# Corv/CUDA-GMM-MPI

Measured on NVIDIA H100. Metric: EM iterations/sec at N=10M D=24 K=64; E-step HBM GB/s vs roofline, higher is better.
Workload: dtype f32

## Files before the change

### cuda-gmm-mpi_b200/csrc/kernels_tc.cu

```cuda
#include <cuda.h>
#include <cudaTypedefs.h>
#include <cuda_fp16.h>
#if defined(__F16C__) && defined(__AVX__)
#include <immintrin.h>
#endif
#include <cuda_runtime.h>

#include <cmath>
#include <cstdio>
#include <cstdlib>
#include <cstring>
#include <string>
#include <vector>

#include "host_math.h"
#include "kernels_tc.cuh"
#include "tc_ptx.cuh"

namespace gmm {

using namespace ptx;

#define TC_CUDA_TRY(expr)                                                                     \
    do {                                                                                      \
        cudaError_t e_ = (expr);                                                              \
        if (e_ != cudaSuccess)                                                                \
            return fail(GMM_ERR_CUDA, std::string(#expr) + ": " + cudaGetErrorString(e_));    \
    } while (0)

constexpr int kTE = 32;
constexpr int kNCL = 32;
constexpr int kNST = 3;
constexpr int kNRAW = 4;
constexpr int kChunkSub = 4;
constexpr int kChunkSub2 = 16;
constexpr int kPhiBits = 11;
constexpr float kGammaScale = 1024.0f;
constexpr float kGammaMagic = 1.5f * 134217728.0f;

template <int D> struct MCfg {
    static_assert(D % 4 == 0, "tensor M-step: D must be a multiple of 4");
    static constexpr int F = 1 + D + D * (D + 1) / 2;
    static constexpr int S = D / 4;
    static constexpr int RPP = 1 + 2 * S + S * (D / 2);
    static constexpr int CPP = (RPP + 7) / 8;
    static constexpr int NCHUNK = 4 * CPP;
    static constexpr int MT = (NCHUNK * 8 + 127) / 128;
    static constexpr int PHI_PART = NCHUNK * 8 * kTE * 2;
    static constexpr int PHI_STAGE = 2 * PHI_PART;
    static constexpr int G_PART = kNCL * kTE * 2;
    static constexpr int G_STAGE = 3 * G_PART;
    static constexpr int RAWX = D * kTE * 4;
    static constexpr int RAWG = kNCL * kTE * 4;
    static constexpr int OFF_PHI = 0;
    static constexpr int OFF_G = OFF_PHI + kNST * PHI_STAGE;
    static constexpr int OFF_RAWX = OFF_G + kNST * G_STAGE;
    static constexpr int OFF_RAWG = OFF_RAWX + kNRAW * RAWX;
    static constexpr int NCT = MT * 128;
    static constexpr int OFF_RACC = OFF_RAWG + kNRAW * RAWG;
    static constexpr int OFF_BAR = OFF_RACC + 32 * NCT * 4;
    static constexpr int SMEM_BYTES = OFF_BAR + 512;
    static constexpr int THREADS = 384 + NCT;
    static constexpr int REG_LAUNCH = (65536 / THREADS) / 8 * 8 > 255 ? 255 : (65536 / THREADS) / 8 * 8;
    static constexpr int REG_P = MT == 1 ? 40 : 24;
    static constexpr int REG_B = MT == 3 ? 80 : 112;
    static constexpr int REG_C = MT == 3 ? 96 : (MT == 2 ? 112 : 240);
    static_assert(128 * REG_P + 256 * REG_B + NCT * REG_C <= THREADS * REG_LAUNCH, "register pools");
    static_assert(OFF_RAWG % 1024 == 0 && RAWG % 1024 == 0, "SWIZZLE_128B TMA destinations need 1024-byte alignment");
    static_assert((MT * 128 - NCHUNK * 8) * kTE * 2 <= kNST * G_STAGE, "the last part's over-read stays inside the operand stages");
    static_assert(MT <= 3, "feature tiles");
};

template <int R, int L>
__device__ __forceinline__ void set_regs() {
    if constexpr (R < L) asm volatile("setmaxnreg.dec.sync.aligned.u32 %0;" ::"n"(R));
    else if constexpr (R > L) asm volatile("setmaxnreg.inc.sync.aligned.u32 %0;" ::"n"(R));
}

struct MMagic { float lin, prod; };

__host__ __device__ constexpr int tri_row(int t) {
    int i = 0;
    while ((i + 1) * (i + 2) / 2 <= t) i++;
    return i;
}

__device__ __forceinline__ void tma_load_2d(void* smem_dst, const CUtensorMap* tmap, int c0, int c1, uint64_t* bar) {
    asm volatile(
        "cp.async.bulk.tensor.2d.shared::cluster.global.mbarrier::complete_tx::bytes [%0], [%1, {%2, %3}], [%4];"
        ::"r"(smem_u32(smem_dst)), "l"(reinterpret_cast<uint64_t>(tmap)), "r"(c0), "r"(c1), "r"(smem_u32(bar)) : "memory");
}

template <int D>
__device__ __forceinline__ void feature_split(const float (&z)[D], int r, const MMagic& mg, float& h, float& l) {
    using C = MCfg<D>;
    if (r == 0) { h = 1.0f; l = 0.0f; }
    else if (r <= C::S) {
        const float v = z[r - 1];
        h = __fsub_rn(__fadd_rn(v, mg.lin), mg.lin);
        l = __fsub_rn(v, h);
    } else if (r < C::RPP) {
        int a, b;
        if (r <= 2 * C::S) { a = r - 1 - C::S; b = a; }
        else { const int t = r - 1 - 2 * C::S; a = t / (D / 2); b = (a + 1 + t % (D / 2)) % D; }
        h = __fsub_rn(__fmaf_rn(z[a], z[b], mg.prod), mg.prod);
        l = __fmaf_rn(z[a], z[b], -h);
    } else { h = 0.0f; l = 0.0f; }
}

template <int D>
__device__ __forceinline__ void build_phi_chunks(const float (&z)[D], const MMagic& mg, uint8_t* hi_base, uint8_t* lo_base, int e, int part) {
    using C = MCfg<D>;
    const int eoff = part * (C::CPP * 512) + (e >> 3) * 128 + (e & 7) * 16;
#pragma unroll
    for (int c = 0; c < C::CPP; c++) {
        float hi[8], lo[8];
#pragma unroll
        for (int u = 0; u < 8; u++) feature_split<D>(z, c * 8 + u, mg, hi[u], lo[u]);
        uint4 h, l;
        h.x = pack_half2(hi[0], hi[1]); h.y = pack_half2(hi[2], hi[3]); h.z = pack_half2(hi[4], hi[5]); h.w = pack_half2(hi[6], hi[7]);
        l.x = pack_half2(lo[0], lo[1]); l.y = pack_half2(lo[2], lo[3]); l.z = pack_half2(lo[4], lo[5]); l.w = pack_half2(lo[6], lo[7]);
        *reinterpret_cast<uint4*>(hi_base + c * 512 + eoff) = h;
        *reinterpret_cast<uint4*>(lo_base + c * 512 + eoff) = l;
    }
}

struct RowInfo { int f, i, j; };
static RowInfo tc_row_info(int D, int row) {
    const int S = D / 4, RPP = 1 + 2 * S + S * (D / 2), CPP = (RPP + 7) / 8;
    const int p = row / (CPP * 8), r = row % (CPP * 8);
    RowInfo o{-1, -1, -1};
    if (p >= 4 || r >= RPP) return o;
    if (r == 0) { if (p == 0) o.f = 0; return o; }
    if (r <= S) { o.i = (r - 1 + p * S) % D; o.f = 1 + o.i; return o; }
    int a, b;
    if (r <= 2 * S) { a = r - 1 - S; b = a; }
    else { const int t = r - 1 - 2 * S; a = t / (D / 2); b = (a + 1 + t % (D / 2)) % D; }
    const int ta = (a + p * S) % D, tb = (b + p * S) % D;
    if (a != b && (b - a + D) % D == D / 2 && ta >= D / 2) return o;
    o.i = ta > tb ? ta : tb;
    o.j = ta > tb ? tb : ta;
    o.f = feat2(D, o.i, o.j);
    return o;
}

__device__ __forceinline__ bool chain_ends(int i, int mt, int nsub) { return ((i + mt) % kChunkSub) == kChunkSub - 1 || i == nsub - 1; }
__device__ __forceinline__ bool chain_starts(int i, int mt) { return i == 0 || ((i + mt) % kChunkSub) == 0; }
__device__ __forceinline__ bool chain2_ends(int i, int mt, int nsub) { return ((i + mt) % kChunkSub2) == kChunkSub2 - 1 || i == nsub - 1; }
__device__ __forceinline__ bool chain2_starts(int i, int mt) { return i == 0 || ((i + mt) % kChunkSub2) == 0; }

template <int D>
__global__ void __launch_bounds__(MCfg<D>::THREADS, 1)
mstep_tc_kernel(const __grid_constant__ CUtensorMap tm_x, const __grid_constant__ CUtensorMap tm_g, int n,
                float* __restrict__ scratch, int events_per_cta, const __grid_constant__ MMagic magic) {
    using C = MCfg<D>;
    extern __shared__ __align__(1024) uint8_t smem[];
    uint64_t* bars = reinterpret_cast<uint64_t*>(smem + C::OFF_BAR);
    uint64_t* raw_full = bars;
    uint64_t* raw_empty = bars + kNRAW;
    uint64_t* op_full = bars + 2 * kNRAW;
    uint64_t* op_empty = op_full + kNST;

    const int warp = threadIdx.x >> 5, lane = threadIdx.x & 31;
    const int e_begin = blockIdx.x * events_per_cta;
    const int e_end = min(n, e_begin + events_per_cta);
    const int nsub = (e_end - e_begin + kTE - 1) / kTE;
    const int k0 = blockIdx.y * kNCL;

    for (int i = threadIdx.x * 16; i < C::OFF_RAWX; i += C::THREADS * 16) *reinterpret_cast<uint4*>(smem + i) = make_uint4(0, 0, 0, 0);
    if (threadIdx.x == 0) {
        for (int s = 0; s < kNRAW; s++) { mbar_init(&raw_full[s], 1); mbar_init(&raw_empty[s], 4); }
        for (int s = 0; s < kNST; s++) { mbar_init(&op_full[s], 4); mbar_init(&op_empty[s], 4 * C::MT); }
        fence_mbar_init();
    }
    fence_proxy_async_smem();
    __syncthreads();

    if (warp < 4) {
        set_regs<C::REG_P, C::REG_LAUNCH>();
        if (warp == 0) {
            if (elect_one()) {
                for (int i = 0; i < nsub; i++) {
                    const int st = i % kNRAW, ph = (i / kNRAW) & 1;
                    mbar_wait_parked(&raw_empty[st], ph ^ 1, 500);
                    mbar_arrive_expect_tx(&raw_full[st], kTE * D * 4 + C::RAWG);
                    const int e0 = e_begin + i * kTE;
                    tma_load_2d(smem + C::OFF_RAWX + st * C::RAWX, &tm_x, e0, 0, &raw_full[st]);
                    tma_load_2d(smem + C::OFF_RAWG + st * C::RAWG, &tm_g, e0, k0, &raw_full[st]);
                }
            }
        }
    } else if (warp < 12) {
        set_regs<C::REG_B, C::REG_LAUNCH>();
        const int bwg = (warp - 4) >> 2;
        const int part = (warp - 4) & 3;
        const int bt = threadIdx.x - 128 - bwg * 128;
        for (int i = bwg; i < nsub; i += 2) {
            const int rs = i % kNRAW, rph = (i / kNRAW) & 1;
            const int os = i % kNST, oph = (i / kNST) & 1;
            mbar_wait_parked(&raw_full[rs], rph, 200);
            float z[D];
            {
                const float* xr = reinterpret_cast<const float*>(smem + C::OFF_RAWX + rs * C::RAWX) + lane;
                int dd = part * C::S;
#pragma unroll
                for (int d = 0; d < D; d++) { z[d] = xr[dd * kTE]; dd = dd + 1 == D ? 0 : dd + 1; }
            }
            uint4 gh, gl, gs;
            float gdep;
            {
                const int kg = bt >> 5, l = bt & 31;
                const int k = kg * 8 + (l & 7), ce = l >> 3;
                const uint8_t* grow = smem + C::OFF_RAWG + rs * C::RAWG + k * (kTE * 4);
                const float4 a = *reinterpret_cast<const float4*>(grow + (((2 * ce) ^ (k & 7)) << 4));
                const float4 b = *reinterpret_cast<const float4*>(grow + (((2 * ce + 1) ^ (k & 7)) << 4));
                const float g[8] = {a.x, a.y, a.z, a.w, b.x, b.y, b.z, b.w};
                gdep = a.x + b.x;
                float hi[8], lo[8];
#pragma unroll
                for (int u = 0; u < 8; u++) {
                    hi[u] = __fsub_rn(__fmaf_rn(g[u], kGammaScale, kGammaMagic), kGammaMagic);
                    lo[u] = __fmaf_rn(g[u], kGammaScale, -hi[u]);
                }
                gh = make_uint4(pack_half2(hi[0], hi[1]), pack_half2(hi[2], hi[3]), pack_half2(hi[4], hi[5]), pack_half2(hi[6], hi[7]));
                gl = make_uint4(pack_half2(lo[0], lo[1]), pack_half2(lo[2], lo[3]), pack_half2(lo[4], lo[5]), pack_half2(lo[6], lo[7]));
                gs = make_uint4(pack_half2(g[0] * kGammaScale, g[1] * kGammaScale), pack_half2(g[2] * kGammaScale, g[3] * kGammaScale),
                                pack_half2(g[4] * kGammaScale, g[5] * kGammaScale), pack_half2(g[6] * kGammaScale, g[7] * kGammaScale));
            }
            float dep = gdep;
#pragma unroll
            for (int d = 0; d < D; d++) dep += z[d];
            __syncwarp();
            if (lane == 0) mbar_arrive_after(&raw_empty[rs], dep);
            else asm volatile("" ::"f"(dep));
            mbar_wait_parked(&op_empty[os], oph ^ 1, 200);
            uint8_t* phi_hi = smem + C::OFF_PHI + os * C::PHI_STAGE;
            uint8_t* phi_lo = phi_hi + C::PHI_PART;
            build_phi_chunks<D>(z, magic, phi_hi, phi_lo, lane, part);
            {
                uint8_t* g_hi = smem + C::OFF_G + os * C::G_STAGE;
                const int kg = bt >> 5, l = bt & 31;
                *reinterpret_cast<uint4*>(g_hi + kg * 512 + l * 16) = gh;
                *reinterpret_cast<uint4*>(g_hi + C::G_PART + kg * 512 + l * 16) = gl;
                *reinterpret_cast<uint4*>(g_hi + 2 * C::G_PART + kg * 512 + l * 16) = gs;
            }
            fence_proxy_async_smem();
            __syncwarp();
            if (lane == 0) mbar_arrive(&op_full[os]);
        }
    } else {
        set_regs<C::REG_C, C::REG_LAUNCH>();
        const int mt = __shfl_sync(0xffffffffu, (warp - 12) >> 2, 0);
        const int ct = threadIdx.x - 384;
        const int wq = warp & 3, gid = lane >> 2, qd = lane & 3;
        float* racc = reinterpret_cast<float*>(smem + C::OFF_RACC) + ct;
#pragma unroll
        for (int j = 0; j < 32; j++) racc[j * C::NCT] = 0.0f;
        float ex[2][16], rm[2][16];
#pragma unroll
        for (int h = 0; h < 2; h++)
#pragma unroll
            for (int j = 0; j < 16; j++) { ex[h][j] = 0.0f; rm[h][j] = 0.0f; }
        int held = -1;
        for (int i = 0; i < nsub; i++) {
            const int os = i % kNST, oph = (i / kNST) & 1;
            mbar_wait_parked(&op_full[os], oph, 100);
            const uint32_t phi = smem_u32(smem + C::OFF_PHI + os * C::PHI_STAGE);
            const uint32_t gam = smem_u32(smem + C::OFF_G + os * C::G_STAGE);
            const bool new1 = chain_starts(i, mt), new2 = chain2_starts(i, mt);
            wgmma_fence();
#pragma unroll
            for (int h = 0; h < 2; h++) {
#pragma unroll
                for (int ks = 0; ks < kTE / 16; ks++) {
                    const uint64_t hdesc = make_smem_desc(gam + ks * 256,  128,  512);
                    const uint64_t ldesc = make_smem_desc(gam + C::G_PART + ks * 256, 128, 512);
                    const uint64_t sdesc = make_smem_desc(gam + 2 * C::G_PART + ks * 256, 128, 512);
                    const uint32_t arow = mt * 8192 + h * 4096 + ks * 256;
                    const uint64_t ah = make_smem_desc(phi + arow,  128,  512);
                    const uint64_t al = make_smem_desc(phi + C::PHI_PART + arow, 128, 512);
                    wgmma_m64n32k16_ss_tn(ex[h], ah, hdesc, ks > 0 || !new1);
                    wgmma_m64n32k16_ss_tn(rm[h], ah, ldesc, ks > 0 || !new2);
                    wgmma_m64n32k16_ss_tn(rm[h], al, sdesc);
                }
            }
            wgmma_commit();
            wgmma_wait<1>();
            __syncwarp();
            if (lane == 0 && held >= 0) mbar_arrive(&op_empty[held]);
            held = os;
            if (chain_ends(i, mt, nsub)) {
                wgmma_wait<0>();
                __syncwarp();
                if (lane == 0) mbar_arrive(&op_empty[os]);
                held = -1;
#pragma unroll
                for (int h = 0; h < 2; h++) {
#pragma unroll
                    for (int j = 0; j < 16; j++) racc[(h * 16 + j) * C::NCT] += ex[h][j];
                    asm volatile("" ::: "memory");
                }
                if (chain2_ends(i, mt, nsub)) {
#pragma unroll
                    for (int h = 0; h < 2; h++) {
#pragma unroll
                        for (int j = 0; j < 16; j++) racc[(h * 16 + j) * C::NCT] += rm[h][j];
                        asm volatile("" ::: "memory");
                    }
                }
            }
        }
        wgmma_wait<0>();
        float* my = scratch + (size_t)(blockIdx.y * gridDim.x + blockIdx.x) * C::MT * 128 * kNCL + (size_t)mt * 128 * kNCL;
#pragma unroll
        for (int h = 0; h < 2; h++)
#pragma unroll
            for (int j = 0; j < 16; j += 2) {
                const int row = h * 64 + wq * 16 + gid + 8 * ((j >> 1) & 1);
                const int col = (j >> 2) * 8 + 2 * qd;
                *reinterpret_cast<float2*>(my + (size_t)row * kNCL + col) =
                    make_float2(racc[(h * 16 + j) * C::NCT], racc[(h * 16 + j + 1) * C::NCT]);
            }
    }
}

__global__ void standardise_soa_kernel(const float* __restrict__ xs, float* __restrict__ zs, size_t pitch, int n, int D,
                                       const float* __restrict__ shift_f, const float* __restrict__ inv_scale_f) {
    const int d = blockIdx.y;
    const float s = shift_f[d], isc = inv_scale_f[d];
    const float* x = xs + (size_t)d * pitch;
    float* z = zs + (size_t)d * pitch;
    for (long long e = (long long)blockIdx.x * blockDim.x + threadIdx.x; e < n; e += (long long)gridDim.x * blockDim.x)
        z[e] = __fmul_rn(__fsub_rn(x[e], s), isc);
}

__global__ void __launch_bounds__(256)
mstep_tc_finalize_kernel(const float* __restrict__ scratch, int ncta_x, int MT, int K, int F, const int3* __restrict__ rowmap,
                         const double* __restrict__ scale, double* __restrict__ stats) {
    constexpr int NQ = 256 / kNCL;
    __shared__ double part[NQ][kNCL];
    const int3 rm = rowmap[blockIdx.x];
    if (rm.x < 0) return;
    const int mt = blockIdx.x / 128, row = blockIdx.x % 128;
    const int col = threadIdx.x & (kNCL - 1), q = threadIdx.x / kNCL;
    double fac = 1.0 / (double)kGammaScale;
    if (rm.y >= 0) fac *= scale[rm.y];
    if (rm.z >= 0) fac *= scale[rm.z];
    for (int ty = 0; ty * kNCL < K; ty++) {
        double s = 0;
        for (int cx = q; cx < ncta_x; cx += NQ)
            s += (double)scratch[(((size_t)(ty * ncta_x + cx) * MT + mt) * 128 + row) * kNCL + col];
        part[q][col] = s;
        __syncthreads();
        const int k = ty * kNCL + col;
        if (q == 0 && k < K) {
            double t = 0;
#pragma unroll
            for (int u = 0; u < NQ; u++) t += part[u][col];
            stats[(size_t)k * F + rm.x] += t * fac;
        }
        __syncthreads();
    }
}


template <int D> struct ECfg {
    static_assert(D % 8 == 0, "tensor E-step: D must be a multiple of 8");
    static constexpr int CP = D / 8;
    static constexpr int NLO = (CP + 1 + 1) / 2 * 2;
    static constexpr int NCHKB = CP + NLO;
    static constexpr int GB = 16;
    static constexpr int N = GB * 8;
    static constexpr int MAXSG = 64 / GB;
    static constexpr int B_BLOCK = NCHKB * N * 16;
    static constexpr int B_SG = CP * B_BLOCK;
    static constexpr int OFF_B = 0;
    static constexpr int OFF_CK = OFF_B + MAXSG * B_SG;
    static constexpr int OFF_SH = OFF_CK + 512;
    static constexpr int OFF_BAR = OFF_SH + 256;
    static constexpr int SMEM_BYTES = OFF_BAR + 64;
    static constexpr int NWG = 2;
    static constexpr int THREADS = 128 * NWG;
};

#ifndef GMM_ESTEP_CUT
#define GMM_ESTEP_CUT 0
#endif

template <int D>
__device__ __forceinline__ void tc_stage_operand(uint8_t* smem, const uint8_t* __restrict__ b_img, const float* __restrict__ ck,
                                                 const float* __restrict__ shift_f, const float* __restrict__ inv_scale_f, int NSG) {
    using C = ECfg<D>;
    uint64_t* b_full = reinterpret_cast<uint64_t*>(smem + C::OFF_BAR);
    float* ck_s = reinterpret_cast<float*>(smem + C::OFF_CK);
    float* sh_s = reinterpret_cast<float*>(smem + C::OFF_SH);
    if (threadIdx.x == 0) { mbar_init(b_full, 1); fence_mbar_init(); }
    if (threadIdx.x < 64) { ck_s[threadIdx.x] = ck[threadIdx.x] * 1.4426950408889634f; ck_s[64 + threadIdx.x] = ck[64 + threadIdx.x]; }
    if (threadIdx.x < D) { sh_s[threadIdx.x] = shift_f[threadIdx.x]; sh_s[32 + threadIdx.x] = inv_scale_f[threadIdx.x]; }
    __syncthreads();
    if (threadIdx.x == 0) {
        mbar_arrive_expect_tx(b_full, (uint32_t)NSG * C::B_SG);
        for (int g = 0; g < NSG * C::CP; g++) tma_load_1d(smem + C::OFF_B + g * C::B_BLOCK, b_img + (size_t)g * C::B_BLOCK, C::B_BLOCK, b_full);
    }
}

template <int D>
__device__ __forceinline__ void tc_split_rows(const float2 (&xa)[D / 8], const float2 (&xb)[D / 8], const float* sh_s, const float* isc_s,
                                              int qd, uint32_t (&zh)[D / 8][2], uint32_t (&zl)[D / 8][2]) {
#pragma unroll
    for (int j = 0; j < D / 8; j++) {
        const float s0 = sh_s[8 * j + 2 * qd], s1 = sh_s[8 * j + 2 * qd + 1];
        const float i0 = isc_s[8 * j + 2 * qd], i1 = isc_s[8 * j + 2 * qd + 1];
#pragma unroll
        for (int r = 0; r < 2; r++) {
            const float2 x = r ? xb[j] : xa[j];
            const float z0 = __fmul_rn(__fsub_rn(x.x, s0), i0), z1 = __fmul_rn(__fsub_rn(x.y, s1), i1);
            const __half2 h = __floats2half2_rn(z0, z1);
            const float2 f = __half22float2(h);
            zh[j][r] = *reinterpret_cast<const uint32_t*>(&h);
            zl[j][r] = pack_half2(z0 - f.x, z1 - f.y);
        }
    }
}

template <int D>
__device__ __forceinline__ void tc_issue_group(float (&acc)[32], const uint32_t (&zh)[D / 8][2], const uint32_t (&zl)[D / 8][2],
                                               uint32_t bsg, int c, int h, uint32_t ones) {
    using C = ECfg<D>;
    constexpr int CP = C::CP;
    constexpr uint32_t CH = C::N * 16;
    const uint32_t bb = bsg + (uint32_t)c * C::B_BLOCK + (uint32_t)h * (CH / 2);
    wgmma_fence();
#pragma unroll
    for (int j = c; j < CP; j++)
        wgmma_m64n64k16_rs(acc, zh[j][0], zh[j][1], zh[j][0], zh[j][1], make_smem_desc(bb + j * CH, CP * CH, 128), j > c);
#pragma unroll
    for (int p = c; p < CP + 1; p += 2) {
        const int x = p, y = p + 1;
        if (y <= CP) {
            const uint32_t yc = y < CP ? (uint32_t)y : 2u * CP;
            const uint32_t a2 = y < CP ? zl[y < CP ? y : 0][0] : ones, a3 = y < CP ? zl[y < CP ? y : 0][1] : ones;
            wgmma_m64n64k16_rs(acc, zl[x][0], zl[x][1], a2, a3, make_smem_desc(bb + x * CH, (yc - x) * CH, 128), true);
        } else {
            wgmma_m64n64k16_rs(acc, 0u, 0u, ones, ones, make_smem_desc(bb + c * CH, (2 * CP - c) * CH, 128), true);
        }
    }
}

template <int D, int NSG>
__device__ __forceinline__ void tc_tile_logits(const uint32_t (&zh)[D / 8][2], const uint32_t (&zl)[D / 8][2], uint32_t bsm,
                                               const float* ck_s, int qd, uint32_t ones, float (&lg)[ECfg<D>::MAXSG][8]) {
    using C = ECfg<D>;
    constexpr int CP = C::CP;
    float acc[2][32];
    tc_issue_group<D>(acc[0], zh, zl, bsm, 0, 0, ones);
    wgmma_commit();
#pragma unroll
    for (int sg = 0; sg < C::MAXSG; sg++) {
        if (sg >= NSG) {
#pragma unroll
            for (int u = 0; u < 8; u++) lg[sg][u] = -INFINITY;
            continue;
        }
        const uint32_t bsg = bsm + (uint32_t)sg * C::B_SG;
        float sq[32];
#pragma unroll
        for (int u = 0; u < 32; u++) sq[u] = 0.f;
#pragma unroll
        for (int c = 0; c < CP; c++) {
#pragma unroll
            for (int h = 0; h < 2; h++) {
                if (sg + 1 == NSG && c + 1 == CP && h == 1) {
                    wgmma_wait<0>();
                } else {
                    if (h == 0) tc_issue_group<D>(acc[1], zh, zl, bsg, c, 1, ones);
                    else if (c + 1 < CP) tc_issue_group<D>(acc[0], zh, zl, bsg, c + 1, 0, ones);
                    else tc_issue_group<D>(acc[0], zh, zl, bsg + C::B_SG, 0, 0, ones);
                    wgmma_commit();
                    wgmma_wait<1>();
                }
                wgmma_pin(acc[h]);
                const float(&a)[32] = acc[h];
#if GMM_ESTEP_CUT == 1
                sq[0] += a[0];
#else
#pragma unroll
                for (int i = 0; i < 8; i++) {
                    float& s0 = sq[16 * h + 2 * i];
                    float& s1 = sq[16 * h + 2 * i + 1];
                    s0 = fmaf(a[4 * i], a[4 * i], fmaf(a[4 * i + 1], a[4 * i + 1], s0));
                    s1 = fmaf(a[4 * i + 2], a[4 * i + 2], fmaf(a[4 * i + 3], a[4 * i + 3], s1));
                }
#endif
            }
        }
#if GMM_ESTEP_CUT == 1
        for (int u = 0; u < 8; u++) lg[sg][u] = sq[0];
        continue;
#endif
        float w[16];
        const bool b1 = qd & 1, b2 = (qd >> 1) & 1;
#pragma unroll
        for (int u = 0; u < 16; u++) {
            const float send = b1 ? sq[u] : sq[16 + u], keep = b1 ? sq[16 + u] : sq[u];
            w[u] = keep + __shfl_xor_sync(0xffffffffu, send, 1);
        }
#pragma unroll
        for (int u = 0; u < 8; u++) {
            const float send = b2 ? w[u] : w[8 + u], keep = b2 ? w[8 + u] : w[u];
            const float qv = keep + __shfl_xor_sync(0xffffffffu, send, 2);
            const int k = sg * C::GB + 8 * (qd & 1) + 4 * (qd >> 1) + (u >> 1);
            lg[sg][u] = fmaf(ck_s[64 + k], qv, ck_s[k]);
        }
    }
}

template <int D, int NSG>
__global__ void __launch_bounds__(ECfg<D>::THREADS, 1)
estep_tc_kernel(const float* __restrict__ x_aos, const uint8_t* __restrict__ b_img, const float* __restrict__ ck,
                const float* __restrict__ shift_f, const float* __restrict__ inv_scale_f, float* __restrict__ memb,
                size_t pitch, int n, int K, double* __restrict__ ll_out, int mode, const float* den_in, float* den_out) {
    using C = ECfg<D>;
    constexpr int CP = C::CP;
    extern __shared__ __align__(1024) uint8_t smem[];
    uint64_t* b_full = reinterpret_cast<uint64_t*>(smem + C::OFF_BAR);
    float* ck_s = reinterpret_cast<float*>(smem + C::OFF_CK);
    float* sh_s = reinterpret_cast<float*>(smem + C::OFF_SH);
    float* isc_s = sh_s + 32;

    const int wg = threadIdx.x >> 7, warp = (threadIdx.x >> 5) & 3, lane = threadIdx.x & 31;
    const int gid = lane >> 2, qd = lane & 3;
    const int ntiles = (n + 63) / 64;

    tc_stage_operand<D>(smem, b_img, ck, shift_f, inv_scale_f, NSG);

    const int r0 = warp * 16 + gid;
    float2 xa[CP], xb[CP];
    auto load_rows = [&](int t) {
        const long long e0 = (long long)t * 64 + r0, e1 = e0 + 8;
#pragma unroll
        for (int j = 0; j < CP; j++) {
            xa[j] = e0 < n ? __ldg(reinterpret_cast<const float2*>(x_aos + (size_t)e0 * D + 8 * j + 2 * qd)) : make_float2(0.f, 0.f);
            xb[j] = e1 < n ? __ldg(reinterpret_cast<const float2*>(x_aos + (size_t)e1 * D + 8 * j + 2 * qd)) : make_float2(0.f, 0.f);
        }
    };
    const int stride = (int)gridDim.x * C::NWG;
    int t = (int)blockIdx.x * C::NWG + wg;
    if (t < ntiles) load_rows(t);
    const uint32_t ones = qd == 0 ? 0x3C003C00u : 0u;
    const uint32_t bsm = smem_u32(smem + C::OFF_B);
    double ll_acc = 0.0;
    constexpr float kLn2 = 0.6931471805599453f;
    mbar_wait(b_full, 0);

    for (; t < ntiles; t += stride) {
        uint32_t zh[CP][2], zl[CP][2];
        tc_split_rows<D>(xa, xb, sh_s, isc_s, qd, zh, zl);
        const long long e0 = (long long)t * 64 + r0, e1 = e0 + 8;
        if (t + stride < ntiles) load_rows(t + stride);

        float lg[C::MAXSG][8];
        tc_tile_logits<D, NSG>(zh, zl, bsm, ck_s, qd, ones, lg);
#if GMM_ESTEP_CUT == 1
        for (int sg = 0; sg < C::MAXSG; sg++) ll_acc += (double)lg[sg][0];
        continue;
#endif
        float mx[2] = {-INFINITY, -INFINITY};
#pragma unroll
        for (int sg = 0; sg < C::MAXSG; sg++)
#pragma unroll
            for (int u = 0; u < 8; u++) mx[u & 1] = fmaxf(mx[u & 1], lg[sg][u]);
#pragma unroll
        for (int r = 0; r < 2; r++) {
            mx[r] = fmaxf(mx[r], __shfl_xor_sync(0xffffffffu, mx[r], 1));
            mx[r] = fmaxf(mx[r], __shfl_xor_sync(0xffffffffu, mx[r], 2));
        }
        float scale[2] = {1.f, 1.f};
        const long long er[2] = {e0, e1};
        if (mode == 3) {
            float d2[2];
#pragma unroll
            for (int r = 0; r < 2; r++) d2[r] = er[r] < n ? den_in[er[r]] * 1.4426950408889634f : 0.f;
#pragma unroll
            for (int sg = 0; sg < C::MAXSG; sg++)
#pragma unroll
                for (int u = 0; u < 8; u++) lg[sg][u] = ex2_approx(lg[sg][u] - d2[u & 1]);
        } else {
            float sm[2] = {0.f, 0.f};
#pragma unroll
            for (int sg = 0; sg < C::MAXSG; sg++)
#pragma unroll
                for (int u = 0; u < 8; u++) { lg[sg][u] = ex2_approx(lg[sg][u] - mx[u & 1]); sm[u & 1] += lg[sg][u]; }
            float dx[2];
#pragma unroll
            for (int r = 0; r < 2; r++) {
                sm[r] += __shfl_xor_sync(0xffffffffu, sm[r], 1);
                sm[r] += __shfl_xor_sync(0xffffffffu, sm[r], 2);
                dx[r] = (mode != 0 && den_in != nullptr && er[r] < n) ? den_in[er[r]] : 0.f;
            }
            __syncwarp();
#pragma unroll
            for (int r = 0; r < 2; r++) {
                float denom = fmaf(mx[r], kLn2, logf(sm[r]));
                scale[r] = 1.0f / sm[r];
                if (mode != 0 && er[r] < n) {
                    if (den_in != nullptr) {
                        const float g = fmaxf(denom, dx[r]);
                        const float tot = g + logf(__expf(denom - g) + __expf(dx[r] - g));
                        scale[r] *= __expf(denom - tot);
                        denom = tot;
                    }
                    if (qd == 0) den_out[er[r]] = denom;
                }
                if (qd == 0 && er[r] < n && (mode == 0 || mode == 2)) ll_acc += (double)denom;
            }
        }
        if (mode != 1 && GMM_ESTEP_CUT != 2) {
#pragma unroll
            for (int sg = 0; sg < C::MAXSG; sg++) {
#pragma unroll
                for (int u = 0; u < 8; u++) {
                    const int k = sg * C::GB + 8 * (qd & 1) + 4 * (qd >> 1) + (u >> 1);
                    const long long e = er[u & 1];
                    if (sg < NSG && (k & ~7) < K && e < n) memb[(size_t)k * pitch + e] = lg[sg][u] * scale[u & 1];
                }
            }
        }
    }
    if (mode == 0 || mode == 2) {
        ll_acc = ll_acc + __shfl_down_sync(0xffffffffu, ll_acc, 16);
        ll_acc = ll_acc + __shfl_down_sync(0xffffffffu, ll_acc, 8);
        ll_acc = ll_acc + __shfl_down_sync(0xffffffffu, ll_acc, 4);
        ll_acc = ll_acc + __shfl_down_sync(0xffffffffu, ll_acc, 2);
        ll_acc = ll_acc + __shfl_down_sync(0xffffffffu, ll_acc, 1);
        if (lane == 0) atomicAdd(ll_out, ll_acc);
    }
}

template <int D, int NSG>
__global__ void __launch_bounds__(ECfg<D>::THREADS, 1)
score_tc_kernel(const float* __restrict__ x_aos, const uint8_t* __restrict__ b_img, const float* __restrict__ ck,
                const float* __restrict__ shift_f, const float* __restrict__ inv_scale_f, int n, int K, int kbase,
                int pass, int last, float* run_den, float* run_bl, int* run_bk, int* __restrict__ labels,
                float* __restrict__ max_resp, float* __restrict__ logp, double* __restrict__ ll_out, int* __restrict__ flag) {
    using C = ECfg<D>;
    constexpr int CP = C::CP;
    extern __shared__ __align__(1024) uint8_t smem[];
    uint64_t* b_full = reinterpret_cast<uint64_t*>(smem + C::OFF_BAR);
    const float* ck_s = reinterpret_cast<const float*>(smem + C::OFF_CK);
    const float* sh_s = reinterpret_cast<const float*>(smem + C::OFF_SH);
    const float* isc_s = sh_s + 32;

    const int wg = threadIdx.x >> 7, warp = (threadIdx.x >> 5) & 3, lane = threadIdx.x & 31;
    const int gid = lane >> 2, qd = lane & 3;
    const int ntiles = (n + 63) / 64;
    tc_stage_operand<D>(smem, b_img, ck, shift_f, inv_scale_f, NSG);

    const int r0 = warp * 16 + gid;
    float2 xa[CP], xb[CP];
    auto load_rows = [&](int t) {
        const long long e0 = (long long)t * 64 + r0, e1 = e0 + 8;
#pragma unroll
        for (int j = 0; j < CP; j++) {
            xa[j] = e0 < n ? __ldg(reinterpret_cast<const float2*>(x_aos + (size_t)e0 * D + 8 * j + 2 * qd)) : make_float2(0.f, 0.f);
            xb[j] = e1 < n ? __ldg(reinterpret_cast<const float2*>(x_aos + (size_t)e1 * D + 8 * j + 2 * qd)) : make_float2(0.f, 0.f);
        }
    };
    const int stride = (int)gridDim.x * C::NWG;
    int t = (int)blockIdx.x * C::NWG + wg;
    if (t < ntiles) load_rows(t);
    const uint32_t ones = qd == 0 ? 0x3C003C00u : 0u;
    const uint32_t bsm = smem_u32(smem + C::OFF_B);
    double ll_acc = 0.0;
    constexpr float kLn2 = 0.6931471805599453f, kLog2e = 1.4426950408889634f;
    bool out_of_range = false;
    mbar_wait(b_full, 0);

    for (; t < ntiles; t += stride) {
        const long long e0 = (long long)t * 64 + r0, e1 = e0 + 8;
#pragma unroll
        for (int j = 0; j < CP; j++)
#pragma unroll
            for (int r = 0; r < 2; r++) {
                const float2 x = r ? xb[j] : xa[j];
                const float z0 = __fmul_rn(__fsub_rn(x.x, sh_s[8 * j + 2 * qd]), isc_s[8 * j + 2 * qd]);
                const float z1 = __fmul_rn(__fsub_rn(x.y, sh_s[8 * j + 2 * qd + 1]), isc_s[8 * j + 2 * qd + 1]);
                out_of_range |= (r ? e1 : e0) < n && (!(fabsf(z0) <= 16384.0f) || !(fabsf(z1) <= 16384.0f));
            }
        uint32_t zh[CP][2], zl[CP][2];
        tc_split_rows<D>(xa, xb, sh_s, isc_s, qd, zh, zl);
        if (t + stride < ntiles) load_rows(t + stride);

        float lg[C::MAXSG][8];
        tc_tile_logits<D, NSG>(zh, zl, bsm, ck_s, qd, ones, lg);

        float mx[2] = {-INFINITY, -INFINITY}, bl[2] = {-INFINITY, -INFINITY};
        int bk[2] = {-1, -1};
#pragma unroll
        for (int sg = 0; sg < C::MAXSG; sg++)
#pragma unroll
            for (int u = 0; u < 8; u++) {
                const float l = lg[sg][u];
                const int k = sg * C::GB + 8 * (qd & 1) + 4 * (qd >> 1) + (u >> 1);
                mx[u & 1] = fmaxf(mx[u & 1], l);
                if (k < K && (l > bl[u & 1] || (bk[u & 1] < 0 && l == l))) { bl[u & 1] = l; bk[u & 1] = kbase + k; }
            }
#pragma unroll
        for (int r = 0; r < 2; r++) {
            mx[r] = fmaxf(mx[r], __shfl_xor_sync(0xffffffffu, mx[r], 1));
            mx[r] = fmaxf(mx[r], __shfl_xor_sync(0xffffffffu, mx[r], 2));
#pragma unroll
            for (int o = 1; o <= 2; o <<= 1) {
                const float ov = __shfl_xor_sync(0xffffffffu, bl[r], o);
                const int ok = __shfl_xor_sync(0xffffffffu, bk[r], o);
                if (ok >= 0 && (bk[r] < 0 || ov > bl[r] || (ov == bl[r] && ok < bk[r]))) { bl[r] = ov; bk[r] = ok; }
            }
        }
        float sm[2] = {0.f, 0.f};
#pragma unroll
        for (int sg = 0; sg < C::MAXSG; sg++)
#pragma unroll
            for (int u = 0; u < 8; u++) sm[u & 1] += ex2_approx(lg[sg][u] - mx[u & 1]);
        const long long er[2] = {e0, e1};
        float dx[2] = {0.f, 0.f}, pbl[2] = {0.f, 0.f};
        int pbk[2] = {-1, -1};
#pragma unroll
        for (int r = 0; r < 2; r++) {
            sm[r] += __shfl_xor_sync(0xffffffffu, sm[r], 1);
            sm[r] += __shfl_xor_sync(0xffffffffu, sm[r], 2);
            if (pass > 0 && er[r] < n) { dx[r] = run_den[er[r]]; pbl[r] = run_bl[er[r]]; pbk[r] = run_bk[er[r]]; }
        }
        __syncwarp();
#pragma unroll
        for (int r = 0; r < 2; r++) {
            float denom = fmaf(mx[r], kLn2, logf(sm[r]));
            float mr = ex2_approx(bl[r] - mx[r]) * (1.0f / sm[r]);
            if (pass > 0) {
                const float g = fmaxf(denom, dx[r]);
                const float tot = g + logf(__expf(denom - g) + __expf(dx[r] - g));
                if (bk[r] >= 0 && (pbk[r] < 0 || bl[r] > pbl[r])) {
                    const float sc = (1.0f / sm[r]) * __expf(denom - tot);
                    mr = ex2_approx(bl[r] - mx[r]) * sc;
                } else {
                    bl[r] = pbl[r]; bk[r] = pbk[r];
                    mr = ex2_approx(bl[r] - __fmul_rn(tot, kLog2e));
                }
                denom = tot;
            }
            if (qd == 0 && er[r] < n) {
                if (last) {
                    labels[er[r]] = bk[r];
                    max_resp[er[r]] = bk[r] >= 0 ? mr : __int_as_float(0x7fc00000);
                    logp[er[r]] = denom;
                    ll_acc += (double)denom;
                } else {
                    run_den[er[r]] = denom; run_bl[er[r]] = bl[r]; run_bk[er[r]] = bk[r];
                }
            }
        }
    }
    if (__any_sync(0xffffffffu, out_of_range) && lane == 0) *flag = 1;
    if (last) {
        ll_acc = ll_acc + __shfl_down_sync(0xffffffffu, ll_acc, 16);
        ll_acc = ll_acc + __shfl_down_sync(0xffffffffu, ll_acc, 8);
        ll_acc = ll_acc + __shfl_down_sync(0xffffffffu, ll_acc, 4);
        ll_acc = ll_acc + __shfl_down_sync(0xffffffffu, ll_acc, 2);
        ll_acc = ll_acc + __shfl_down_sync(0xffffffffu, ll_acc, 1);
        if (lane == 0) atomicAdd(ll_out, ll_acc);
    }
}

struct TcState {
    const float* d_x = nullptr;
    const float* d_x_soa = nullptr;
    float* d_z_soa = nullptr;
    float* d_memb = nullptr;
    size_t memb_pitch = 0;
    int n = 0, D = 0, Kmax = 0, num_sms = 132;
    CUtensorMap tm_x{}, tm_g{};
    bool maps_ok = false;
    float* d_shift_f = nullptr;
    float* d_inv_scale_f = nullptr;
    double* d_scale = nullptr;
    float* d_scratch = nullptr;
    size_t scratch_floats = 0;
    bool have_shift = false;
    bool mstep_ready = false;
    float zmax[GMM_MAX_DIMENSIONS] = {0};
    MMagic magic{0.f, 0.f};
    int3* d_rowmap = nullptr;
    CUtensorMap tm_cx{}, tm_cg{};
    const void* cmap_z = nullptr;
    const void* cmap_g = nullptr;
    size_t cmap_pitch = 0;
    int cmap_n = -1;
    CUtensorMap tm_x128{};
    bool emap_ok = false;
    uint8_t* d_bimg = nullptr;
    uint8_t* h_bimg = nullptr;
    size_t bimg_bytes = 0;
    uint8_t* d_opnd = nullptr;
    uint8_t* h_opnd = nullptr;
    cudaEvent_t ev_h2d = nullptr;
    bool h2d_pending = false;
    float* d_ck = nullptr;
    float* h_ck = nullptr;
    float* d_den = nullptr;
    int e_ck_len = 0;
    int e_NG = 0;
    int host_threads = 8;
    bool attr_estep = false, attr_mstep = false, attr_score = false;
    double h_shift[GMM_MAX_DIMENSIONS] = {0}, h_scale[GMM_MAX_DIMENSIONS] = {0};
};

static PFN_cuTensorMapEncodeTiled_v12000 encode_fn() {
    static PFN_cuTensorMapEncodeTiled_v12000 fn = nullptr;
    static bool tried = false;
    if (!tried) {
        tried = true;
        void* p = nullptr;
        cudaDriverEntryPointQueryResult q;
        if (cudaGetDriverEntryPoint("cuTensorMapEncodeTiled", &p, cudaEnableDefault, &q) == cudaSuccess && q == cudaDriverEntryPointSuccess)
            fn = reinterpret_cast<PFN_cuTensorMapEncodeTiled_v12000>(p);
    }
    return fn;
}

static int make_map_2d(CUtensorMap* m, const void* base, uint64_t dim0, uint64_t dim1, uint64_t stride1_bytes, uint32_t box0, uint32_t box1,
                       bool swizzle128 = false) {
    auto fn = encode_fn();
    if (!fn) return fail(GMM_ERR_CUDA, "cuTensorMapEncodeTiled not available from the driver");
    cuuint64_t dims[2] = {dim0, dim1};
    cuuint64_t strides[1] = {stride1_bytes};
    cuuint32_t box[2] = {box0, box1};
    cuuint32_t estr[2] = {1, 1};
    CUresult r = fn(m, CU_TENSOR_MAP_DATA_TYPE_FLOAT32, 2, const_cast<void*>(base), dims, strides, box, estr,
                    CU_TENSOR_MAP_INTERLEAVE_NONE, swizzle128 ? CU_TENSOR_MAP_SWIZZLE_128B : CU_TENSOR_MAP_SWIZZLE_NONE, CU_TENSOR_MAP_L2_PROMOTION_L2_128B,
                    CU_TENSOR_MAP_FLOAT_OOB_FILL_NONE);
    if (r != CUDA_SUCCESS) return fail(GMM_ERR_CUDA, "cuTensorMapEncodeTiled failed (" + std::to_string((int)r) + ")");
    return GMM_OK;
}

bool tc_mstep_supported(int D, int K) {
    (void)K;
    return D == 4 || D == 8 || D == 12 || D == 16 || D == 20 || D == 24;
}
bool tc_estep_supported(int D, int K) { return (D == 8 || D == 16 || D == 24) && K >= 1 && K <= GMM_MAX_CLUSTERS; }

template <int D> static size_t ecfg_pass_bytes() { return (size_t)ECfg<D>::MAXSG * ECfg<D>::B_SG; }
static size_t pass_bytes_for(int D) {
    switch (D) { case 8: return ecfg_pass_bytes<8>(); case 16: return ecfg_pass_bytes<16>(); case 24: return ecfg_pass_bytes<24>(); default: return 0; }
}

int tc_create(TcState** out, const float* d_x_aos, const float* d_x_soa, int n, int D, int Kmax, float* d_memb, size_t memb_pitch, int num_sms,
              cudaStream_t stream) {
    (void)stream;
    TcState* t = new TcState();
    t->d_x = d_x_aos; t->d_x_soa = d_x_soa; t->d_memb = d_memb; t->memb_pitch = memb_pitch; t->n = n; t->D = D; t->Kmax = Kmax; t->num_sms = num_sms;
    *out = t;
    if (n <= 0 || !tc_mstep_supported(D, Kmax)) return GMM_OK;
    TC_CUDA_TRY(cudaMalloc(&t->d_shift_f, sizeof(float) * GMM_MAX_DIMENSIONS));
    TC_CUDA_TRY(cudaMalloc(&t->d_inv_scale_f, sizeof(float) * GMM_MAX_DIMENSIONS));
    TC_CUDA_TRY(cudaMalloc(&t->d_scale, sizeof(double) * GMM_MAX_DIMENSIONS));
    TC_CUDA_TRY(cudaMalloc(&t->d_z_soa, sizeof(float) * memb_pitch * D));
    if (int rc = make_map_2d(&t->tm_x, t->d_z_soa, (uint64_t)n, (uint64_t)D, (uint64_t)memb_pitch * 4, kTE, (uint32_t)D)) return rc;
    if (int rc = make_map_2d(&t->tm_g, d_memb, (uint64_t)n, (uint64_t)Kmax, (uint64_t)memb_pitch * 4, kTE, kNCL, true)) return rc;
    t->maps_ok = true;
    if (D == 8 || D == 16 || D == 24) {
        const int passes = (Kmax + 63) / 64;
        t->e_ck_len = passes * 64;
        t->bimg_bytes = (size_t)passes * pass_bytes_for(D);
        const size_t ck_bytes = sizeof(float) * 2 * t->e_ck_len;
        TC_CUDA_TRY(cudaMalloc(&t->d_opnd, ck_bytes + t->bimg_bytes));
        TC_CUDA_TRY(cudaMallocHost(&t->h_opnd, ck_bytes + t->bimg_bytes));
        t->d_ck = reinterpret_cast<float*>(t->d_opnd);
        t->h_ck = reinterpret_cast<float*>(t->h_opnd);
        t->d_bimg = t->d_opnd + ck_bytes;
        t->h_bimg = t->h_opnd + ck_bytes;
        TC_CUDA_TRY(cudaEventCreateWithFlags(&t->ev_h2d, cudaEventDisableTiming));
        if (passes > 1) TC_CUDA_TRY(cudaMalloc(&t->d_den, sizeof(float) * memb_pitch));
        t->emap_ok = true;
    }
    const int rpp = 1 + 2 * (D / 4) + (D / 4) * (D / 2), nrows = 4 * ((rpp + 7) / 8) * 8;
    const int mt = (nrows + 127) / 128;
    {
        std::vector<int3> rm((size_t)mt * 128);
        std::vector<char> seen((size_t)num_features(D), 0);
        for (int row = 0; row < mt * 128; row++) {
            const RowInfo ri = tc_row_info(D, row);
            rm[row] = make_int3(ri.f, ri.i, ri.j);
            if (ri.f >= 0) {
                if (seen[ri.f]) return fail(GMM_ERR_STATE, "tensor M-step row map: a statistic is produced twice");
                seen[ri.f] = 1;
            }
        }
        for (char c : seen) if (!c) return fail(GMM_ERR_STATE, "tensor M-step row map: a statistic is not produced");
        TC_CUDA_TRY(cudaMalloc(&t->d_rowmap, sizeof(int3) * rm.size()));
        TC_CUDA_TRY(cudaMemcpy(t->d_rowmap, rm.data(), sizeof(int3) * rm.size(), cudaMemcpyHostToDevice));
    }
    const int ytiles = (Kmax + kNCL - 1) / kNCL;
    t->scratch_floats = (size_t)num_sms * ytiles * mt * 128 * kNCL;
    TC_CUDA_TRY(cudaMalloc(&t->d_scratch, sizeof(float) * t->scratch_floats));
    return GMM_OK;
}

void tc_set_host_threads(TcState* t, int n) { if (t) t->host_threads = n < 1 ? 1 : n; }
bool tc_mstep_ready(const TcState* t) { return t && t->maps_ok && t->have_shift && t->mstep_ready; }
bool tc_estep_range_ok(const TcState* t) {
    if (!t || !t->have_shift) return false;
    for (int d = 0; d < t->D; d++)
        if (!(t->zmax[d] <= 16384.0f)) return false;
    return true;
}

void tc_destroy(TcState* t) {
    if (!t) return;
    cudaFree(t->d_shift_f); cudaFree(t->d_inv_scale_f); cudaFree(t->d_scale); cudaFree(t->d_scratch);
    cudaFree(t->d_opnd); cudaFree(t->d_den); cudaFree(t->d_z_soa); cudaFree(t->d_rowmap);
    if (t->h_opnd) cudaFreeHost(t->h_opnd);
    if (t->ev_h2d) cudaEventDestroy(t->ev_h2d);
    delete t;
}

int tc_set_shift_scale(TcState* t, double* shift, const double* scale, const double* xmin, const double* xmax, cudaStream_t stream) {
    if (!t || !t->maps_ok) return GMM_OK;
    float sf[GMM_MAX_DIMENSIONS] = {0}, isf[GMM_MAX_DIMENSIONS] = {0};
    double sc[GMM_MAX_DIMENSIONS] = {0};
    for (int d = 0; d < t->D; d++) {
        sf[d] = (float)shift[d];
        shift[d] = (double)sf[d];
        const double s = (scale && scale[d] > 0) ? scale[d] : 1.0;
        isf[d] = (float)(1.0 / s);
        sc[d] = 1.0 / (double)isf[d];
        t->h_shift[d] = shift[d];
        t->h_scale[d] = sc[d];
        const double za = std::fmax(std::fabs(xmax[d] - (double)sf[d]), std::fabs(xmin[d] - (double)sf[d])) * (double)isf[d] * (1.0 + 1e-6);
        int e2 = 0;
        if (za > 0 && std::isfinite(za)) { e2 = std::ilogb(za) + 1; }
        t->zmax[d] = std::isfinite(za) ? (float)std::ldexp(1.0, e2) : INFINITY;
    }
    {
        float zb = 0.f;
        for (int d = 0; d < t->D; d++) zb = std::fmax(zb, t->zmax[d]);
        t->mstep_ready = zb <= 64.0f;
        const double q = (double)zb / (double)(1 << kPhiBits);
        t->magic.lin = (float)(1.5 * 8388608.0 * q);
        t->magic.prod = (float)(1.5 * 8388608.0 * q * (double)zb);
    }
    TC_CUDA_TRY(cudaMemcpyAsync(t->d_shift_f, sf, sizeof(sf), cudaMemcpyHostToDevice, stream));
    TC_CUDA_TRY(cudaMemcpyAsync(t->d_inv_scale_f, isf, sizeof(isf), cudaMemcpyHostToDevice, stream));
    TC_CUDA_TRY(cudaMemcpyAsync(t->d_scale, sc, sizeof(sc), cudaMemcpyHostToDevice, stream));
    {
        dim3 grid((unsigned)std::min<long long>(4LL * t->num_sms, ((long long)t->n + 255) / 256), (unsigned)t->D);
        standardise_soa_kernel<<<grid, 256, 0, stream>>>(t->d_x_soa, t->d_z_soa, t->memb_pitch, t->n, t->D, t->d_shift_f, t->d_inv_scale_f);
        TC_CUDA_TRY(cudaGetLastError());
    }
    TC_CUDA_TRY(cudaStreamSynchronize(stream));
    t->have_shift = true;
    return GMM_OK;
}


static inline uint16_t f2h_bits(float f) {
    uint32_t x;
    std::memcpy(&x, &f, 4);
    const uint32_t sign = (x >> 16) & 0x8000u;
    x &= 0x7fffffffu;
    if (x >= 0x47800000u) return (uint16_t)(sign | 0x7c00u);
    if (x < 0x38800000u) {
        float a;
        std::memcpy(&a, &x, 4);
        return (uint16_t)(sign | (uint32_t)lrintf(a * 16777216.0f));
    }
    x += ((x >> 13) & 1u) + 0xfffu;
    return (uint16_t)(sign | ((x - 0x38000000u) >> 13));
}
static inline float h2f_bits(uint16_t h) {
    const uint32_t sign = (uint32_t)(h & 0x8000u) << 16;
    const uint32_t em = h & 0x7fffu;
    float r;
    if (em >= 0x0400u) {
        const uint32_t x = sign | ((em << 13) + 0x38000000u);
        std::memcpy(&r, &x, 4);
    } else {
        r = (float)em * (1.0f / 16777216.0f);
        if (sign) r = -r;
    }
    return r;
}

template <int D>
static int bimg_cluster(TcState* t, const clusters_t* host, int k, int K, const double* Wext = nullptr) {
    using C = ECfg<D>;
    int bad = 0;
    {
        const int sg = k / C::GB, i = k % C::GB;
        auto rowp = [&](int d, int chunk) -> uint16_t* {
            const int c = d / 8, ncol = i * 8 + (d % 8);
            return reinterpret_cast<uint16_t*>(t->h_bimg + ((size_t)sg * C::CP + c) * C::B_BLOCK + (size_t)chunk * C::N * 16 + (size_t)ncol * 16);
        };
        if (k >= K) {
            for (int d = 0; d < D; d++)
                for (int c = 0; c < C::NCHKB; c++) std::memset(rowp(d, c), 0, 16);
            return 0;
        }
        double A[D][D], Gc[D][D];
        const float* Ri = host->Rinv + (size_t)k * D * D;
        bool ok = true;
        if (Wext) {
            for (int r = 0; r < D; r++)
                for (int j = 0; j < D; j++) Gc[r][j] = Wext[j * D + r];
        } else {
            for (int r = 0; r < D; r++)
                for (int j = 0; j < D; j++) { A[r][j] = 0.5 * ((double)Ri[r * D + j] + (double)Ri[j * D + r]); Gc[r][j] = 0.0; }
        }
        for (int j = 0; j < D && !Wext; j++) {
            const double d = A[j][j];
            if (!(d > 0.0) || !std::isfinite(d)) { ok = false; break; }
            const double piv = std::sqrt(d), rp = 1.0 / piv;
            Gc[j][j] = piv;
            for (int r = j + 1; r < D; r++) Gc[r][j] = A[r][j] * rp;
            for (int r = j + 1; r < D; r++) {
                const double l = Gc[r][j];
                for (int cc = j + 1; cc <= r; cc++) A[r][cc] -= l * Gc[cc][j];
            }
        }
        if (!ok) return 1;
        alignas(32) float wrow[D][D];
        double vd[D];
        float amax = 0.f;
        for (int d = 0; d < D; d++) {
            double v = 0.0;
            for (int j = 0; j < D; j++) {
                const double w = (j >= d) ? Gc[j][d] : 0.0;
                v = std::fma(-w, (double)host->means[(size_t)k * D + j] - t->h_shift[j], v);
                wrow[d][j] = (float)(w * t->h_scale[j]);
                amax = std::fmax(amax, std::fabs(wrow[d][j]));
            }
            vd[d] = v;
            amax = std::fmax(amax, (float)std::fabs(v));
        }
        if (!std::isfinite(amax)) return 2;
        int e2 = amax > 0.f ? 12 - std::ilogb(amax) : 0;
        e2 = e2 > 40 ? 40 : (e2 < -40 ? -40 : e2);
        for (int d = 0; d < D; d++) {
            for (int j = 0; j < D; j++) wrow[d][j] = std::ldexp(wrow[d][j], e2);
            vd[d] = std::ldexp(vd[d], e2);
            for (int c = 0; c < C::CP; c++) {
                uint16_t *ph = rowp(d, c), *pl = rowp(d, C::CP + c);
#if defined(__F16C__) && defined(__AVX__)
                const __m256 w8 = _mm256_load_ps(&wrow[d][8 * c]);
                const __m128i h8 = _mm256_cvtps_ph(w8, _MM_FROUND_TO_NEAREST_INT | _MM_FROUND_NO_EXC);
                const __m256 l8 = _mm256_sub_ps(w8, _mm256_cvtph_ps(h8));
                _mm_storeu_si128(reinterpret_cast<__m128i*>(ph), h8);
                _mm_storeu_si128(reinterpret_cast<__m128i*>(pl), _mm256_cvtps_ph(l8, _MM_FROUND_TO_NEAREST_INT | _MM_FROUND_NO_EXC));
#else
                for (int e = 0; e < 8; e++) {
                    const uint16_t wh = f2h_bits(wrow[d][8 * c + e]);
                    ph[e] = wh;
                    pl[e] = f2h_bits(wrow[d][8 * c + e] - h2f_bits(wh));
                }
#endif
            }
            const float vf = (float)vd[d];
            if (!(std::fabs(vf) < 6.0e4f)) bad = 2;
            uint16_t* pv = rowp(d, 2 * C::CP);
            const uint16_t vh = f2h_bits(vf);
            std::memset(pv, 0, 16);
            pv[0] = vh;
            pv[1] = f2h_bits((float)(vd[d] - (double)h2f_bits(vh)));
            if (C::NCHKB > 2 * C::CP + 1) std::memset(rowp(d, 2 * C::CP + 1), 0, 16);
        }
        float* ckp = t->h_ck + (size_t)(k / 64) * 128 + (k % 64);
        ckp[0] = host->constant[k] + (float)std::log((double)host->pi[k]);
        ckp[64] = (float)std::ldexp(-0.5 * 1.4426950408889634, -2 * e2);
    }
    return bad;
}

static int bimg_cluster_any(TcState* t, const clusters_t* host, int k, int K, const double* Wext = nullptr) {
    switch (t->D) {
        case 8: return bimg_cluster<8>(t, host, k, K, Wext);
        case 16: return bimg_cluster<16>(t, host, k, K, Wext);
        case 24: return bimg_cluster<24>(t, host, k, K, Wext);
        default: return 3;
    }
}

int tc_params_begin(TcState* t, int K, cudaStream_t stream) {
    if (!t || !t->emap_ok) return fail(GMM_ERR_STATE, "tensor E-step not initialised for this shape");
    if (!t->have_shift) return fail(GMM_ERR_STATE, "tensor E-step needs the global moments (shift/scale) first");
    (void)stream;
    if (t->h2d_pending) {
        TC_CUDA_TRY(cudaEventSynchronize(t->ev_h2d));
        t->h2d_pending = false;
    }
    for (int k = K; k < t->e_ck_len; k++) {
        float* ckp = t->h_ck + (size_t)(k / 64) * 128 + (k % 64);
        ckp[0] = -1e30f;
        ckp[64] = 0.f;
    }
    return GMM_OK;
}
int tc_params_padded(const TcState*, int K) { return (K + 15) / 16 * 16; }
int tc_params_cluster(TcState* t, const clusters_t* host, int k, int K) { return bimg_cluster_any(t, host, k, K); }
int tc_params_cluster_w(TcState* t, const clusters_t* host, int k, int K, const double* W) { return bimg_cluster_any(t, host, k, K, W); }
int tc_params_commit(TcState* t, int K, int bad, cudaStream_t stream) {
    if (bad == 1) return fail(GMM_ERR_STATE, "tensor E-step: inverse covariance of a cluster is not positive definite");
    if (bad == 2) return fail(GMM_ERR_STATE, "tensor E-step: whitening factor exceeds the FP16 range");
    if (bad) return fail(GMM_ERR_ARG, "tensor E-step: unsupported D");
    t->e_NG = (K + 15) / 16;
    const size_t used = (size_t)t->e_NG * (pass_bytes_for(t->D) / 4);
    TC_CUDA_TRY(cudaMemcpyAsync(t->d_opnd, t->h_opnd, sizeof(float) * 2 * t->e_ck_len + used, cudaMemcpyHostToDevice, stream));
    TC_CUDA_TRY(cudaEventRecord(t->ev_h2d, stream));
    t->h2d_pending = true;
    return GMM_OK;
}


int tc_upload_params(TcState* t, const clusters_t* host, int K, cudaStream_t stream) {
    if (int rc = tc_params_begin(t, K, stream)) return rc;
    const int kp = tc_params_padded(t, K);
    const int nt = t->host_threads;
    int bad = 0;
    (void)nt;
#pragma omp parallel for schedule(static) num_threads(nt) reduction(max : bad) if (nt > 1 && K >= 8)
    for (int k = 0; k < kp; k++) {
        const int b = tc_params_cluster(t, host, k, K);
        bad = b > bad ? b : bad;
    }
    return tc_params_commit(t, K, bad, stream);
}

__host__ __device__ inline size_t pset_off_means(int Kmax) { return 3 * (size_t)Kmax; }
__host__ __device__ inline size_t pset_off_R(int Kmax, int D) { return pset_off_means(Kmax) + (size_t)Kmax * D; }
__host__ __device__ inline size_t pset_off_Rinv(int Kmax, int D) { return pset_off_R(Kmax, D) + (size_t)Kmax * D * D; }

#ifdef GMM_FIN_PROF
#define FIN_STAMP(i) do { if (k == 0 && tid == 0) fin_t[i] = clock64(); } while (0)
#else
#define FIN_STAMP(i) do { } while (0)
#endif

template <int D> struct FinCfg { static constexpr int T = (D * D > 256 ? (D * D + 31) / 32 * 32 : 256), NW = T / 32; };

template <int D>
__global__ void __launch_bounds__(FinCfg<D>::T)
finalize_params_kernel(const double* __restrict__ stats, const float* __restrict__ avgvar, const float* __restrict__ shift_f,
                       const double* __restrict__ scale, float* __restrict__ set, int Kmax, int K, int kp,
                       uint8_t* __restrict__ bimg, float* __restrict__ ck, double* __restrict__ ll_out, int* __restrict__ bad, int iter,
                       int fault_iter) {
#ifdef GMM_FIN_PROF
    long long fin_t[10];
#endif
    using C = ECfg<D>;
    constexpr int T = FinCfg<D>::T, NW = FinCfg<D>::NW;
    constexpr int F = 1 + D + D * (D + 1) / 2;
    constexpr int LD = D + 1;
    const int k = blockIdx.x, tid = threadIdx.x;
    if (bad[0] >= 0) return;
    float* ckp = ck + (size_t)(k / 64) * 128 + (k % 64);
    const int sg = k / C::GB, ci = k % C::GB;
    auto rowp = [&](int d, int chunk) -> uint8_t* {
        return bimg + ((size_t)sg * C::CP + d / 8) * C::B_BLOCK + (size_t)chunk * C::N * 16 + (size_t)(ci * 8 + d % 8) * 16;
    };
    if (k >= K) {
        if (tid == 0) { ckp[0] = -1e30f; ckp[64] = 0.f; }
        if (k < kp)
            for (int idx = tid; idx < D * C::NCHKB; idx += T) *reinterpret_cast<uint4*>(rowp(idx / C::NCHKB, idx % C::NCHKB)) = make_uint4(0u, 0u, 0u, 0u);
        return;
    }
    FIN_STAMP(0);
    __shared__ double sS[F + 3], sA[D][LD], sU[D][LD], sW[D][LD], sdm[D], sscale[D], svd[D], sredd[NW];
    __shared__ float swr[D][LD], sredf[NW];
    __shared__ int sbad;
    const double* s = stats + (size_t)k * F;
    for (int f = tid; f < F; f += T) sS[f] = s[f];
    double part = 0.0;
    for (int kk = tid; kk < K; kk += T) part += (double)(float)stats[(size_t)kk * F];
    double shift_d = 0.0;
    if (tid < D) { shift_d = (double)shift_f[tid]; sscale[tid] = scale[tid]; }
    const float av = avgvar[k];
    double ll_slot = 0.0;
    if (k == 0 && tid == 0) ll_slot = stats[(size_t)K * F];
#pragma unroll
    for (int o = 16; o > 0; o >>= 1) part += __shfl_xor_sync(0xffffffffu, part, o);
    if ((tid & 31) == 0) sredd[tid >> 5] = part;
    if (tid == 0) sbad = 0;
    __syncthreads();
    FIN_STAMP(1);
    const double S0 = sS[0];
    const float Nf = (float)S0;
    if (k == 0 && tid == 0) {
        *ll_out = ll_slot;
        if (isnan(S0)) atomicMax(&sbad, 4);
        if (iter == fault_iter) atomicMax(&sbad, 1);
    }
    double sumN = 0.0;
#pragma unroll
    for (int w = 0; w < NW; w++) sumN += sredd[w];
    const float pik = Nf < 0.5f ? 1e-10f : (float)((double)Nf / sumN);
    if (tid < D) {
        const double m = (S0 != 0.0) ? sS[1 + tid] / S0 : 0.0;
        const float mu = (Nf > 0.5f) ? (float)(m + shift_d) : 0.0f;
        sdm[tid] = (double)mu - shift_d;
        set[pset_off_means(Kmax) + (size_t)k * D + tid] = mu;
    }
    {
        float* R = set + pset_off_R(Kmax, D) + (size_t)k * D * D;
        const double inv = 1.0 / (double)Nf;
        for (int idx = tid; idx < D * D; idx += T) {
            const int i = idx / D, j = idx % D;
            if (j > i) continue;
            float v;
            if (Nf > 0.5f) {
                const double mi = (S0 != 0.0) ? sS[1 + i] / S0 : 0.0;
                double cov = (Nf >= 1.0f) ? sS[1 + D + i * (i + 1) / 2 + j] - mi * sS[1 + j] : 0.0;
                if (i == j) cov += av;
                v = (float)(cov * inv);
            } else {
                v = (i == j) ? 1.0f : 0.0f;
            }
            R[i * D + j] = v; R[j * D + i] = v;
            sA[j][i] = (double)v;
            if (i == j) sW[i][i] = 0.0; else { sW[j][i] = 0.0; sW[i][j] = 0.0; }
        }
    }
    __syncthreads();
    FIN_STAMP(2);
    bool ok = true;
    for (int j = D - 1; j >= 0; j--) {
        double d = sA[j][j];
        for (int m = j + 1; m < D; m++) d = __dsub_rn(d, __dmul_rn(sU[j][m], sU[j][m]));
        if (!(d > 0.0) || !isfinite(d)) { ok = false; break; }
        const double piv = sqrt(d), rp = 1.0 / piv;
        if (tid < j) {
            double v = sA[tid][j];
            for (int m = j + 1; m < D; m++) v = __dsub_rn(v, __dmul_rn(sU[tid][m], sU[j][m]));
            sU[tid][j] = __dmul_rn(v, rp);
        } else if (tid == j) {
            sU[j][j] = piv;
        }
        __syncthreads();
    }
    if (!ok) {
        if (tid == 0) { atomicCAS(&bad[0], -1, iter); atomicMax(&bad[1], 1); }
        return;
    }
    FIN_STAMP(3);
    if (tid < D) {
        const int j = tid;
        for (int i = D - 1; i > j; i--) sW[i][j] = 0.0;
        sW[j][j] = 1.0 / sU[j][j];
        for (int i = j - 1; i >= 0; i--) {
            double v = 0.0;
            for (int m = i + 1; m <= j; m++) v = __dsub_rn(v, __dmul_rn(sU[i][m], sW[m][j]));
            sW[i][j] = v / sU[i][i];
        }
    }
    __syncthreads();
    FIN_STAMP(4);
    {
        float* Ri = set + pset_off_Rinv(Kmax, D) + (size_t)k * D * D;
        for (int idx = tid; idx < D * D; idx += T) {
            const int i = idx / D, j = idx % D;
            if (j < i) continue;
            double v = 0.0;
#pragma unroll 4
            for (int m = 0; m <= i; m++) v = __dadd_rn(v, __dmul_rn(sW[m][i], sW[m][j]));
            Ri[i * D + j] = (float)v; Ri[j * D + i] = (float)v;
        }
    }
    FIN_STAMP(5);
    float amax = 0.f;
    for (int idx = tid; idx < D * D; idx += T) {
        const int d = idx / D, j = idx % D;
        const float w = (j >= d) ? (float)(sW[d][j] * sscale[j]) : 0.f;
        swr[d][j] = w;
        amax = fmaxf(amax, fabsf(w));
    }
    if (tid >= 64 && tid < 64 + D) {
        const int d = tid - 64;
        double v = 0.0;
#pragma unroll 4
        for (int j = d; j < D; j++) v = fma(-sW[d][j], sdm[j], v);
        svd[d] = v;
        amax = fmaxf(amax, (float)fabs(v));
    }
    if (tid == 32) {
        double ld = 0.0;
        for (int j = D - 1; j >= 0; j--) ld += log(sU[j][j]);
        sredd[0] = ld;
    }
#pragma unroll
    for (int o = 16; o > 0; o >>= 1) amax = fmaxf(amax, __shfl_xor_sync(0xffffffffu, amax, o));
    if ((tid & 31) == 0) sredf[tid >> 5] = amax;
    __syncthreads();
    FIN_STAMP(6);
    const double ld = sredd[0];
    const float cst = (float)(-D * 0.5 * log(2.0 * 3.1415926535897931) - 0.5 * (2.0 * ld));
    if (tid == 0) { set[k] = Nf; set[Kmax + k] = pik; set[2 * (size_t)Kmax + k] = cst; }
    amax = 0.f;
#pragma unroll
    for (int w = 0; w < NW; w++) amax = fmaxf(amax, sredf[w]);
    if (!isfinite(amax)) {
        if (tid == 0) { atomicCAS(&bad[0], -1, iter); atomicMax(&bad[1], 2); }
        return;
    }
    int e2 = amax > 0.f ? 12 - ilogbf(amax) : 0;
    e2 = e2 > 40 ? 40 : (e2 < -40 ? -40 : e2);
    for (int idx = tid; idx < D * C::CP; idx += T) {
        const int d = idx / C::CP, c = idx % C::CP;
        uint32_t hi[4], lo[4];
#pragma unroll
        for (int e = 0; e < 4; e++) {
            const float w0 = ldexpf(swr[d][8 * c + 2 * e], e2), w1 = ldexpf(swr[d][8 * c + 2 * e + 1], e2);
            const __half2 h = __floats2half2_rn(w0, w1);
            const float2 hf = __half22float2(h);
            hi[e] = *reinterpret_cast<const uint32_t*>(&h);
            lo[e] = pack_half2(w0 - hf.x, w1 - hf.y);
        }
        *reinterpret_cast<uint4*>(rowp(d, c)) = make_uint4(hi[0], hi[1], hi[2], hi[3]);
        *reinterpret_cast<uint4*>(rowp(d, C::CP + c)) = make_uint4(lo[0], lo[1], lo[2], lo[3]);
    }
    if (tid >= 128 && tid < 128 + D) {
        const int d = tid - 128;
        const double vs = ldexp(svd[d], e2);
        const float vf = (float)vs;
        if (!(fabsf(vf) < 6.0e4f)) atomicMax(&sbad, 2);
        const __half vh = __float2half_rn(vf);
        const __half vl = __float2half_rn((float)(vs - (double)__half2float(vh)));
        const uint32_t p = (uint32_t)__half_as_ushort(vh) | ((uint32_t)__half_as_ushort(vl) << 16);
        *reinterpret_cast<uint4*>(rowp(d, 2 * C::CP)) = make_uint4(p, 0u, 0u, 0u);
        if (C::NCHKB > 2 * C::CP + 1) *reinterpret_cast<uint4*>(rowp(d, 2 * C::CP + 1)) = make_uint4(0u, 0u, 0u, 0u);
    }
    if (tid == 0) {
        ckp[0] = cst + (float)log((double)pik);
        ckp[64] = (float)ldexp(-0.5 * 1.4426950408889634, -2 * e2);
    }
    __syncthreads();
    FIN_STAMP(7);
#ifdef GMM_FIN_PROF
    if (k == 0 && tid == 0)
        printf("fin phases (cycles): stage %lld  means+R %lld  cholesky %lld  inverse %lld  Rinv %lld  rows+v+log %lld  operand %lld\n",
               fin_t[1] - fin_t[0], fin_t[2] - fin_t[1], fin_t[3] - fin_t[2], fin_t[4] - fin_t[3], fin_t[5] - fin_t[4], fin_t[6] - fin_t[5], fin_t[7] - fin_t[6]);
#endif
    if (tid == 0 && sbad) { atomicCAS(&bad[0], -1, iter); atomicMax(&bad[1], sbad); }
}

size_t tc_param_set_floats(int Kmax, int D) { return (size_t)Kmax * (3 + (size_t)D + 2 * (size_t)D * D); }
size_t tc_param_set_off(int Kmax, int D, int which) {
    switch (which) {
        case 0: return 0;
        case 1: return (size_t)Kmax;
        case 2: return 2 * (size_t)Kmax;
        case 3: return pset_off_means(Kmax);
        case 4: return pset_off_R(Kmax, D);
        default: return pset_off_Rinv(Kmax, D);
    }
}
bool tc_finalize_supported(const TcState* t, int K) {
    return t && t->emap_ok && t->have_shift && tc_estep_supported(t->D, K) && tc_estep_range_ok(t);
}
int tc_launch_finalize(TcState* t, int K, const double* d_stats, const float* d_avgvar, float* d_set, double* d_ll, int* d_bad, int iter,
                       int fault_iter, cudaStream_t stream) {
    if (!tc_finalize_supported(t, K)) return fail(GMM_ERR_STATE, "device-side finalisation not available for this state");
    const int kp = tc_params_padded(t, K);
    const int grid = ((K + 63) / 64) * 64;
#define GMM_FIN(d) finalize_params_kernel<d><<<grid, FinCfg<d>::T, 0, stream>>>(d_stats, d_avgvar, t->d_shift_f, t->d_scale, d_set, t->Kmax, K, kp, \
                                                                     t->d_bimg, t->d_ck, d_ll, d_bad, iter, fault_iter)
    switch (t->D) {
        case 8: GMM_FIN(8); break;
        case 16: GMM_FIN(16); break;
        case 24: GMM_FIN(24); break;
        default: return fail(GMM_ERR_ARG, "device-side finalisation: unsupported D");
    }
#undef GMM_FIN
    TC_CUDA_TRY(cudaGetLastError());
    t->e_NG = (K + 15) / 16;
    return GMM_OK;
}

template <int D>
static int launch_estep_d(TcState* t, int K, const float* x, int n, float* memb, size_t pitch, float* den, double* d_ll, cudaStream_t stream) {
    using C = ECfg<D>;
    static_assert(C::SMEM_BYTES <= 232448, "shared memory budget");
    static void (*const kern[C::MAXSG])(const float*, const uint8_t*, const float*, const float*, const float*, float*, size_t, int, int,
                                        double*, int, const float*, float*) = {estep_tc_kernel<D, 1>, estep_tc_kernel<D, 2>,
                                                                              estep_tc_kernel<D, 3>, estep_tc_kernel<D, 4>};
    static_assert(C::MAXSG == 4, "one kernel instance per supergroup count");
    if (!t->attr_estep) {
        for (auto* k : kern) TC_CUDA_TRY(cudaFuncSetAttribute(k, cudaFuncAttributeMaxDynamicSharedMemorySize, C::SMEM_BYTES));
        t->attr_estep = true;
    }
    const int ntiles = (n + 127) / 128;
    int grid = t->num_sms;
    if (grid > ntiles) grid = ntiles;
    if (grid < 1) grid = 1;
    const int NP = (K + 63) / 64;
    if (NP > 1 && !den) return fail(GMM_ERR_STATE, "tensor E-step: context was created for at most 64 clusters");
    auto launch = [&](int p, int mode, const float* den_in, float* den_out) {
        const int Kp = K - 64 * p < 64 ? K - 64 * p : 64;
        kern[(Kp + C::GB - 1) / C::GB - 1]<<<grid, C::THREADS, C::SMEM_BYTES, stream>>>(
            x, t->d_bimg + (size_t)p * C::MAXSG * C::B_SG, t->d_ck + 128 * p, t->d_shift_f, t->d_inv_scale_f,
            memb + (size_t)(64 * p) * pitch, pitch, n, Kp, d_ll, mode, den_in, den_out);
        return cudaGetLastError();
    };
    if (NP == 1) TC_CUDA_TRY(launch(0, 0, nullptr, nullptr));
    else {
        for (int p = 0; p + 1 < NP; p++) TC_CUDA_TRY(launch(p, 1, p ? den : nullptr, den));
        TC_CUDA_TRY(launch(NP - 1, 2, den, den));
        for (int p = 0; p + 1 < NP; p++) TC_CUDA_TRY(launch(p, 3, den, nullptr));
    }
    return GMM_OK;
}

static int launch_estep_any(TcState* t, int K, const float* x, int n, float* memb, size_t pitch, float* den, double* d_ll, cudaStream_t stream) {
    if (!t || !t->emap_ok) return fail(GMM_ERR_STATE, "tensor E-step not initialised for this shape");
    switch (t->D) {
        case 8: return launch_estep_d<8>(t, K, x, n, memb, pitch, den, d_ll, stream);
        case 16: return launch_estep_d<16>(t, K, x, n, memb, pitch, den, d_ll, stream);
        case 24: return launch_estep_d<24>(t, K, x, n, memb, pitch, den, d_ll, stream);
        default: return fail(GMM_ERR_ARG, "tensor E-step: unsupported D");
    }
}

int tc_launch_estep(TcState* t, int K, double* d_ll, cudaStream_t stream) {
    if (!t) return fail(GMM_ERR_STATE, "tensor E-step not initialised for this shape");
    return launch_estep_any(t, K, t->d_x, t->n, t->d_memb, t->memb_pitch, t->d_den, d_ll, stream);
}

int tc_launch_estep_on(TcState* t, int K, const float* d_x_aos, int n, float* d_memb, size_t pitch, float* d_den, double* d_ll,
                       cudaStream_t stream) {
    if (n <= 0) return GMM_OK;
    return launch_estep_any(t, K, d_x_aos, n, d_memb, pitch, d_den, d_ll, stream);
}

template <int D>
static int launch_score_d(TcState* t, int K, const TcScoreIo& io, cudaStream_t stream) {
    using C = ECfg<D>;
    static void (*const kern[C::MAXSG])(const float*, const uint8_t*, const float*, const float*, const float*, int, int, int, int, int,
                                        float*, float*, int*, int*, float*, float*, double*, int*) = {
        score_tc_kernel<D, 1>, score_tc_kernel<D, 2>, score_tc_kernel<D, 3>, score_tc_kernel<D, 4>};
    static_assert(C::MAXSG == 4, "one kernel instance per supergroup count");
    if (!t->attr_score) {
        for (auto* k : kern) TC_CUDA_TRY(cudaFuncSetAttribute(k, cudaFuncAttributeMaxDynamicSharedMemorySize, C::SMEM_BYTES));
        t->attr_score = true;
    }
    const int ntiles = (io.n + 127) / 128;
    int grid = t->num_sms;
    if (grid > ntiles) grid = ntiles;
    if (grid < 1) grid = 1;
    const int NP = (K + 63) / 64;
    if (NP > 1 && !(io.run_den && io.run_bl && io.run_bk)) return fail(GMM_ERR_STATE, "tensor scoring: no running state for K > 64");
    for (int p = 0; p < NP; p++) {
        const int Kp = K - 64 * p < 64 ? K - 64 * p : 64;
        kern[(Kp + C::GB - 1) / C::GB - 1]<<<grid, C::THREADS, C::SMEM_BYTES, stream>>>(
            io.x, t->d_bimg + (size_t)p * C::MAXSG * C::B_SG, t->d_ck + 128 * p, t->d_shift_f, t->d_inv_scale_f, io.n, Kp, 64 * p, p, p + 1 == NP, io.run_den, io.run_bl, io.run_bk, io.labels, io.max_resp, io.logp, io.ll,
            io.flag);
        TC_CUDA_TRY(cudaGetLastError());
    }
    return GMM_OK;
}

int tc_launch_score(TcState* t, int K, const TcScoreIo& io, cudaStream_t stream) {
    if (!t || !t->emap_ok) return fail(GMM_ERR_STATE, "tensor scoring not initialised for this shape");
    if (io.n <= 0) return GMM_OK;
    switch (t->D) {
        case 8: return launch_score_d<8>(t, K, io, stream);
        case 16: return launch_score_d<16>(t, K, io, stream);
        case 24: return launch_score_d<24>(t, K, io, stream);
        default: return fail(GMM_ERR_ARG, "tensor scoring: unsupported D");
    }
}

template <int D>
static int launch_mstep_d(TcState* t, int K, const CUtensorMap& tm_x, const CUtensorMap& tm_g, int n, double* d_stats, cudaStream_t stream) {
    using C = MCfg<D>;
    static_assert(C::SMEM_BYTES <= 232448, "shared memory budget");
    if (!t->attr_mstep) {
        TC_CUDA_TRY(cudaFuncSetAttribute(mstep_tc_kernel<D>, cudaFuncAttributeMaxDynamicSharedMemorySize, C::SMEM_BYTES));
        t->attr_mstep = true;
    }
    int gx = t->num_sms;
    int per = (n + gx - 1) / gx;
    per = (per + kTE - 1) / kTE * kTE;
    gx = (n + per - 1) / per;
    const int gy = (K + kNCL - 1) / kNCL;
    if ((size_t)gx * gy * C::MT * 128 * kNCL > t->scratch_floats) return fail(GMM_ERR_STATE, "tensor M-step scratch too small");
    dim3 grid(gx, gy);
    mstep_tc_kernel<D><<<grid, C::THREADS, C::SMEM_BYTES, stream>>>(tm_x, tm_g, n, t->d_scratch, per, t->magic);
    TC_CUDA_TRY(cudaGetLastError());
    mstep_tc_finalize_kernel<<<C::NCHUNK * 8, 256, 0, stream>>>(t->d_scratch, gx, C::MT, K, C::F, t->d_rowmap, t->d_scale, d_stats);
    TC_CUDA_TRY(cudaGetLastError());
    return GMM_OK;
}

static int launch_mstep_any(TcState* t, int K, const CUtensorMap& tm_x, const CUtensorMap& tm_g, int n, double* d_stats, cudaStream_t stream) {
    if (!t || !t->maps_ok) return fail(GMM_ERR_STATE, "tensor-core M-step not initialised for this shape");
    if (!t->have_shift) return fail(GMM_ERR_STATE, "tensor-core M-step needs gmm_seed (shift/scale) first");
    if (!t->mstep_ready) return fail(GMM_ERR_STATE, "tensor-core M-step: the data range exceeds the fixed-point operand budget");
    switch (t->D) {
        case 4: return launch_mstep_d<4>(t, K, tm_x, tm_g, n, d_stats, stream);
        case 8: return launch_mstep_d<8>(t, K, tm_x, tm_g, n, d_stats, stream);
        case 12: return launch_mstep_d<12>(t, K, tm_x, tm_g, n, d_stats, stream);
        case 16: return launch_mstep_d<16>(t, K, tm_x, tm_g, n, d_stats, stream);
        case 20: return launch_mstep_d<20>(t, K, tm_x, tm_g, n, d_stats, stream);
        case 24: return launch_mstep_d<24>(t, K, tm_x, tm_g, n, d_stats, stream);
        default: return fail(GMM_ERR_ARG, "tensor-core M-step: unsupported D");
    }
}

int tc_launch_mstep(TcState* t, int K, double* d_stats, cudaStream_t stream) {
    if (!t) return fail(GMM_ERR_STATE, "tensor-core M-step not initialised for this shape");
    return launch_mstep_any(t, K, t->tm_x, t->tm_g, t->n, d_stats, stream);
}

int tc_launch_mstep_on(TcState* t, int K, const float* d_z, const float* d_memb, size_t pitch, int n, double* d_stats, cudaStream_t stream) {
    if (n <= 0) return GMM_OK;
    if (!t || !t->maps_ok) return fail(GMM_ERR_STATE, "tensor-core M-step not initialised for this shape");
    if (t->cmap_z != d_z || t->cmap_g != d_memb || t->cmap_pitch != pitch || t->cmap_n != n) {
        t->cmap_n = -1;
        if (int rc = make_map_2d(&t->tm_cx, d_z, (uint64_t)n, (uint64_t)t->D, (uint64_t)pitch * 4, kTE, (uint32_t)t->D)) return rc;
        if (int rc = make_map_2d(&t->tm_cg, d_memb, (uint64_t)n, (uint64_t)t->Kmax, (uint64_t)pitch * 4, kTE, kNCL, true)) return rc;
        t->cmap_z = d_z; t->cmap_g = d_memb; t->cmap_pitch = pitch; t->cmap_n = n;
    }
    return launch_mstep_any(t, K, t->tm_cx, t->tm_cg, n, d_stats, stream);
}

const float* tc_shift_f(const TcState* t) { return t && t->have_shift ? t->d_shift_f : nullptr; }
const float* tc_inv_scale_f(const TcState* t) { return t && t->have_shift ? t->d_inv_scale_f : nullptr; }
float tc_mstep_zbound(const TcState* t) {
    float zb = 0.f;
    if (t)
        for (int d = 0; d < t->D; d++) zb = std::fmax(zb, t->zmax[d]);
    return zb;
}

}
```

### cuda-gmm-mpi_b200/csrc/tc_ptx.cuh

```cuda
#pragma once
#include <cuda_runtime.h>
#include <cstdint>

namespace gmm { namespace ptx {

__device__ __forceinline__ uint32_t smem_u32(const void* p) {
    return static_cast<uint32_t>(__cvta_generic_to_shared(p));
}

__device__ __forceinline__ void mbar_init(uint64_t* bar, uint32_t count) {
    asm volatile("mbarrier.init.shared::cta.b64 [%0], %1;" ::"r"(smem_u32(bar)), "r"(count) : "memory");
}
__device__ __forceinline__ void fence_mbar_init() {
    asm volatile("fence.mbarrier_init.release.cluster;" ::: "memory");
}
__device__ __forceinline__ void mbar_arrive(uint64_t* bar) {
    asm volatile("mbarrier.arrive.shared::cta.b64 _, [%0];" ::"r"(smem_u32(bar)) : "memory");
}
__device__ __forceinline__ void mbar_arrive_after(uint64_t* bar, float dep) {
    asm volatile(
        "{\n\t.reg .pred p;\n\t.reg .b32 cnt;\n\t"
        "setp.ne.b32 p, %1, 0xff800001;\n\t"
        "selp.b32 cnt, 1, 2, p;\n\t"
        "mbarrier.arrive.shared::cta.b64 _, [%0], cnt;\n\t}"
        ::"r"(smem_u32(bar)), "r"(__float_as_uint(dep)) : "memory");
}
__device__ __forceinline__ void mbar_arrive_expect_tx(uint64_t* bar, uint32_t bytes) {
    asm volatile("mbarrier.arrive.expect_tx.shared::cta.b64 _, [%0], %1;" ::"r"(smem_u32(bar)), "r"(bytes) : "memory");
}
__device__ __forceinline__ bool mbar_try_wait(uint64_t* bar, uint32_t parity) {
    uint32_t ok;
    asm volatile(
        "{\n\t.reg .pred p;\n\t"
        "mbarrier.try_wait.parity.shared::cta.b64 p, [%1], %2;\n\t"
        "selp.u32 %0, 1, 0, p;\n\t}"
        : "=r"(ok) : "r"(smem_u32(bar)), "r"(parity) : "memory");
    return ok != 0;
}
__device__ __forceinline__ void mbar_wait(uint64_t* bar, uint32_t parity) {
    while (!mbar_try_wait(bar, parity)) {}
}
__device__ __forceinline__ void mbar_wait_parked(uint64_t* bar, uint32_t parity, uint32_t ns) {
    uint32_t ok = 0;
    while (!ok) {
        asm volatile(
            "{\n\t.reg .pred p;\n\t"
            "mbarrier.try_wait.parity.shared::cta.b64 p, [%1], %2, %3;\n\t"
            "selp.u32 %0, 1, 0, p;\n\t}"
            : "=r"(ok) : "r"(smem_u32(bar)), "r"(parity), "r"(ns) : "memory");
    }
}
__device__ __forceinline__ void fence_proxy_async_smem() {
    asm volatile("fence.proxy.async.shared::cta;" ::: "memory");
}

__device__ __forceinline__ void tma_load_1d(void* smem_dst, const void* gmem_src, uint32_t bytes, uint64_t* bar) {
    asm volatile(
        "cp.async.bulk.shared::cluster.global.mbarrier::complete_tx::bytes [%0], [%1], %2, [%3];"
        ::"r"(smem_u32(smem_dst)), "l"(gmem_src), "r"(bytes), "r"(smem_u32(bar)) : "memory");
}

__device__ __forceinline__ uint64_t make_smem_desc(uint32_t saddr, uint32_t lbo_bytes, uint32_t sbo_bytes) {
    uint64_t d = 0;
    d |= (uint64_t)((saddr >> 4) & 0x3FFF);
    d |= (uint64_t)((lbo_bytes >> 4) & 0x3FFF) << 16;
    d |= (uint64_t)((sbo_bytes >> 4) & 0x3FFF) << 32;
    return d;
}

__device__ __forceinline__ void wgmma_fence() { asm volatile("wgmma.fence.sync.aligned;" ::: "memory"); }
__device__ __forceinline__ void wgmma_commit() { asm volatile("wgmma.commit_group.sync.aligned;" ::: "memory"); }
__device__ __forceinline__ void wgmma_wait_all() { asm volatile("wgmma.wait_group.sync.aligned 0;" ::: "memory"); }
template <int N>
__device__ __forceinline__ void wgmma_wait() { asm volatile("wgmma.wait_group.sync.aligned %0;" ::"n"(N) : "memory"); }
template <int N>
__device__ __forceinline__ void wgmma_pin(float (&d)[N]) {
#pragma unroll
    for (int i = 0; i < N; i++) asm volatile("" : "+f"(d[i])::"memory");
}

__device__ __forceinline__ void wgmma_m64n64k16_rs(float (&d)[32], uint32_t a0, uint32_t a1, uint32_t a2, uint32_t a3, uint64_t b_desc, bool accumulate) {
    asm volatile(
        "{\n\t.reg .pred p;\n\t"
        "setp.ne.b32 p, %37, 0;\n\t"
        "wgmma.mma_async.sync.aligned.m64n64k16.f32.f16.f16 "
        "{%0, %1, %2, %3, %4, %5, %6, %7, %8, %9, %10, %11, %12, %13, %14, %15, %16, %17, %18, %19, %20, %21, %22, %23, %24, %25, %26, %27, %28, %29, %30, %31}, "
        "{%32, %33, %34, %35}, %36, p, 1, 1, 0;\n\t}"
        : "+f"(d[0]), "+f"(d[1]), "+f"(d[2]), "+f"(d[3]), "+f"(d[4]), "+f"(d[5]), "+f"(d[6]), "+f"(d[7]), "+f"(d[8]), "+f"(d[9]), "+f"(d[10]), "+f"(d[11]), "+f"(d[12]), "+f"(d[13]), "+f"(d[14]), "+f"(d[15]), "+f"(d[16]), "+f"(d[17]), "+f"(d[18]), "+f"(d[19]), "+f"(d[20]), "+f"(d[21]), "+f"(d[22]), "+f"(d[23]), "+f"(d[24]), "+f"(d[25]), "+f"(d[26]), "+f"(d[27]), "+f"(d[28]), "+f"(d[29]), "+f"(d[30]), "+f"(d[31])
        : "r"(a0), "r"(a1), "r"(a2), "r"(a3), "l"(b_desc), "r"((uint32_t)accumulate));
}

__device__ __forceinline__ void wgmma_m64n32k16_ss_tn(float (&d)[16], uint64_t a_desc, uint64_t b_desc, bool accumulate = true) {
    asm volatile(
        "{\n\t.reg .pred p;\n\t"
        "setp.ne.b32 p, %18, 0;\n\t"
        "wgmma.mma_async.sync.aligned.m64n32k16.f32.f16.f16 "
        "{%0, %1, %2, %3, %4, %5, %6, %7, %8, %9, %10, %11, %12, %13, %14, %15}, "
        "%16, %17, p, 1, 1, 1, 0;\n\t}"
        : "+f"(d[0]), "+f"(d[1]), "+f"(d[2]), "+f"(d[3]), "+f"(d[4]), "+f"(d[5]), "+f"(d[6]), "+f"(d[7]), "+f"(d[8]), "+f"(d[9]), "+f"(d[10]), "+f"(d[11]), "+f"(d[12]), "+f"(d[13]), "+f"(d[14]), "+f"(d[15])
        : "l"(a_desc), "l"(b_desc), "r"((uint32_t)accumulate));
}

__device__ __forceinline__ bool elect_one() {
    uint32_t pred;
    asm volatile(
        "{\n\t.reg .pred p;\n\t"
        "elect.sync _|p, 0xffffffff;\n\t"
        "selp.u32 %0, 1, 0, p;\n\t}"
        : "=r"(pred));
    return pred != 0;
}

__device__ __forceinline__ uint32_t pack_half2(float a, float b) {
    uint32_t r;
    asm("cvt.rn.f16x2.f32 %0, %1, %2;" : "=r"(r) : "f"(b), "f"(a));
    return r;
}

__device__ __forceinline__ float ex2_approx(float x) {
    float r;
    asm("ex2.approx.ftz.f32 %0, %1;" : "=f"(r) : "f"(x));
    return r;
}

}}
```

Measured before the change: 120.5.

## Build M-step feature operands in registers inside consumer warpgroups, dropping builder warps

Removes the separate phi-builder warpgroups and the shared-memory phi staging buffers. Consumer warpgroups now compute the hi/lo fp16 split of the outer-product features directly in registers from the raw x tile, using a host-computed operand map. They feed those registers to register-sourced wgmma m64n32k16. Gamma conversion moves into the producer warpgroup's spare warps, and register budgets are retuned. This is meant to cut shared-memory traffic and inter-warpgroup synchronization, at the cost of more per-consumer ALU work, register pressure and a complex host-side row layout.

```diff
diff --git a/cuda-gmm-mpi_b200/csrc/kernels_tc.cu b/cuda-gmm-mpi_b200/csrc/kernels_tc.cu
--- a/cuda-gmm-mpi_b200/csrc/kernels_tc.cu
+++ b/cuda-gmm-mpi_b200/csrc/kernels_tc.cu
@@ -15,6 +15,7 @@
 
 #include "host_math.h"
 #include "kernels_tc.cuh"
+#include "mstep_rows.h"
 #include "tc_ptx.cuh"
 
 namespace gmm {
@@ -42,32 +43,26 @@
     static_assert(D % 4 == 0, "tensor M-step: D must be a multiple of 4");
     static constexpr int F = 1 + D + D * (D + 1) / 2;
     static constexpr int S = D / 4;
-    static constexpr int RPP = 1 + 2 * S + S * (D / 2);
-    static constexpr int CPP = (RPP + 7) / 8;
-    static constexpr int NCHUNK = 4 * CPP;
-    static constexpr int MT = (NCHUNK * 8 + 127) / 128;
-    static constexpr int PHI_PART = NCHUNK * 8 * kTE * 2;
-    static constexpr int PHI_STAGE = 2 * PHI_PART;
+    static constexpr int MT = (4 * ((1 + 2 * S + S * (D / 2) + 7) / 8) * 8 + 127) / 128;
     static constexpr int G_PART = kNCL * kTE * 2;
     static constexpr int G_STAGE = 3 * G_PART;
-    static constexpr int RAWX = D * kTE * 4;
+    static constexpr int RAWZ = (D * kTE * 4 + 1023) / 1024 * 1024;
+    static constexpr int RAWX = RAWZ + 1024;
     static constexpr int RAWG = kNCL * kTE * 4;
-    static constexpr int OFF_PHI = 0;
-    static constexpr int OFF_G = OFF_PHI + kNST * PHI_STAGE;
+    static constexpr int OFF_G = 0;
     static constexpr int OFF_RAWX = OFF_G + kNST * G_STAGE;
     static constexpr int OFF_RAWG = OFF_RAWX + kNRAW * RAWX;
     static constexpr int NCT = MT * 128;
     static constexpr int OFF_RACC = OFF_RAWG + kNRAW * RAWG;
     static constexpr int OFF_BAR = OFF_RACC + 32 * NCT * 4;
     static constexpr int SMEM_BYTES = OFF_BAR + 512;
-    static constexpr int THREADS = 384 + NCT;
+    static constexpr int THREADS = 128 + NCT;
     static constexpr int REG_LAUNCH = (65536 / THREADS) / 8 * 8 > 255 ? 255 : (65536 / THREADS) / 8 * 8;
-    static constexpr int REG_P = MT == 1 ? 40 : 24;
-    static constexpr int REG_B = MT == 3 ? 80 : 112;
-    static constexpr int REG_C = MT == 3 ? 96 : (MT == 2 ? 112 : 240);
-    static_assert(128 * REG_P + 256 * REG_B + NCT * REG_C <= THREADS * REG_LAUNCH, "register pools");
+    static constexpr int REG_P = MT == 1 ? REG_LAUNCH : 56;
+    static constexpr int REG_C = MT == 3 ? 152 : (MT == 2 ? 224 : REG_LAUNCH);
+    static_assert(128 * REG_P + NCT * REG_C <= THREADS * REG_LAUNCH, "register pools");
+    static_assert(OFF_RAWX % 1024 == 0 && RAWX % 1024 == 0 && RAWZ % 1024 == 0, "SWIZZLE_128B TMA destinations need 1024-byte alignment");
     static_assert(OFF_RAWG % 1024 == 0 && RAWG % 1024 == 0, "SWIZZLE_128B TMA destinations need 1024-byte alignment");
-    static_assert((MT * 128 - NCHUNK * 8) * kTE * 2 <= kNST * G_STAGE, "the last part's over-read stays inside the operand stages");
     static_assert(MT <= 3, "feature tiles");
 };
 
@@ -79,69 +74,72 @@
 
 struct MMagic { float lin, prod; };
 
-__host__ __device__ constexpr int tri_row(int t) {
-    int i = 0;
-    while ((i + 1) * (i + 2) / 2 <= t) i++;
-    return i;
-}
-
 __device__ __forceinline__ void tma_load_2d(void* smem_dst, const CUtensorMap* tmap, int c0, int c1, uint64_t* bar) {
     asm volatile(
         "cp.async.bulk.tensor.2d.shared::cluster.global.mbarrier::complete_tx::bytes [%0], [%1, {%2, %3}], [%4];"
         ::"r"(smem_u32(smem_dst)), "l"(reinterpret_cast<uint64_t>(tmap)), "r"(c0), "r"(c1), "r"(smem_u32(bar)) : "memory");
 }
 
-template <int D>
-__device__ __forceinline__ void feature_split(const float (&z)[D], int r, const MMagic& mg, float& h, float& l) {
-    using C = MCfg<D>;
-    if (r == 0) { h = 1.0f; l = 0.0f; }
-    else if (r <= C::S) {
-        const float v = z[r - 1];
-        h = __fsub_rn(__fadd_rn(v, mg.lin), mg.lin);
-        l = __fsub_rn(v, h);
-    } else if (r < C::RPP) {
-        int a, b;
-        if (r <= 2 * C::S) { a = r - 1 - C::S; b = a; }
-        else { const int t = r - 1 - 2 * C::S; a = t / (D / 2); b = (a + 1 + t % (D / 2)) % D; }
-        h = __fsub_rn(__fmaf_rn(z[a], z[b], mg.prod), mg.prod);
-        l = __fmaf_rn(z[a], z[b], -h);
-    } else { h = 0.0f; l = 0.0f; }
-}
-
-template <int D>
-__device__ __forceinline__ void build_phi_chunks(const float (&z)[D], const MMagic& mg, uint8_t* hi_base, uint8_t* lo_base, int e, int part) {
-    using C = MCfg<D>;
-    const int eoff = part * (C::CPP * 512) + (e >> 3) * 128 + (e & 7) * 16;
-#pragma unroll
-    for (int c = 0; c < C::CPP; c++) {
-        float hi[8], lo[8];
-#pragma unroll
-        for (int u = 0; u < 8; u++) feature_split<D>(z, c * 8 + u, mg, hi[u], lo[u]);
-        uint4 h, l;
-        h.x = pack_half2(hi[0], hi[1]); h.y = pack_half2(hi[2], hi[3]); h.z = pack_half2(hi[4], hi[5]); h.w = pack_half2(hi[6], hi[7]);
-        l.x = pack_half2(lo[0], lo[1]); l.y = pack_half2(lo[2], lo[3]); l.z = pack_half2(lo[4], lo[5]); l.w = pack_half2(lo[6], lo[7]);
-        *reinterpret_cast<uint4*>(hi_base + c * 512 + eoff) = h;
-        *reinterpret_cast<uint4*>(lo_base + c * 512 + eoff) = l;
-    }
-}
-
-struct RowInfo { int f, i, j; };
-static RowInfo tc_row_info(int D, int row) {
-    const int S = D / 4, RPP = 1 + 2 * S + S * (D / 2), CPP = (RPP + 7) / 8;
-    const int p = row / (CPP * 8), r = row % (CPP * 8);
-    RowInfo o{-1, -1, -1};
-    if (p >= 4 || r >= RPP) return o;
-    if (r == 0) { if (p == 0) o.f = 0; return o; }
-    if (r <= S) { o.i = (r - 1 + p * S) % D; o.f = 1 + o.i; return o; }
-    int a, b;
-    if (r <= 2 * S) { a = r - 1 - S; b = a; }
-    else { const int t = r - 1 - 2 * S; a = t / (D / 2); b = (a + 1 + t % (D / 2)) % D; }
-    const int ta = (a + p * S) % D, tb = (b + p * S) % D;
-    if (a != b && (b - a + D) % D == D / 2 && ta >= D / 2) return o;
-    o.i = ta > tb ? ta : tb;
-    o.j = ta > tb ? tb : ta;
-    o.f = feat2(D, o.i, o.j);
-    return o;
+__device__ __forceinline__ float2 lds_f2(uint32_t addr) {
+    float2 v;
+    asm volatile("ld.shared.v2.f32 {%0, %1}, [%2];" : "=f"(v.x), "=f"(v.y) : "r"(addr) : "memory");
+    return v;
+}
+
+__device__ __forceinline__ void feature_split(float a, float b, float m, float& h, float& l) {
+    h = __fsub_rn(__fmaf_rn(a, b, m), m);
+    l = __fmaf_rn(a, b, -h);
+}
+
+#ifndef GMM_MSTEP_CUT
+#define GMM_MSTEP_CUT 0
+#endif
+
+__device__ __forceinline__ void build_half(const float2 (&za)[4], const float2 (&zb0)[4], const float2 (&zb1)[4], float m0, float m1,
+                                           uint32_t (&hi)[2][4], uint32_t (&lo)[2][4]) {
+#pragma unroll
+    for (int p = 0; p < 4; p++) {
+        const int ks = p >> 1, u = p & 1;
+#if GMM_MSTEP_CUT == 2
+        hi[ks][2 * u] = __float_as_uint(zb0[p].x); hi[ks][2 * u + 1] = __float_as_uint(zb1[p].x);
+        lo[ks][2 * u] = __float_as_uint(zb0[p].y); lo[ks][2 * u + 1] = __float_as_uint(zb1[p].y);
+        (void)za; (void)m0; (void)m1;
+#else
+        float h0, l0, h1, l1, h2, l2, h3, l3;
+        feature_split(za[p].x, zb0[p].x, m0, h0, l0);
+        feature_split(za[p].y, zb0[p].y, m0, h1, l1);
+        feature_split(za[p].x, zb1[p].x, m1, h2, l2);
+        feature_split(za[p].y, zb1[p].y, m1, h3, l3);
+        hi[ks][2 * u] = pack_half2(h0, h1);
+        hi[ks][2 * u + 1] = pack_half2(h2, h3);
+        lo[ks][2 * u] = pack_half2(l0, l1);
+        lo[ks][2 * u + 1] = pack_half2(l2, l3);
+#endif
+    }
+}
+
+__device__ __forceinline__ void load_row(uint32_t addr, float2 (&z)[4]) {
+#pragma unroll
+    for (int p = 0; p < 4; p++) z[p] = lds_f2(addr ^ (uint32_t)(p << 5));
+}
+
+__device__ __forceinline__ void issue_half(float (&ex)[16], float (&rm)[16], const uint32_t (&hi)[2][4], const uint32_t (&lo)[2][4],
+                                           uint32_t gam, bool new1, bool new2) {
+#pragma unroll
+    for (int ks = 0; ks < kTE / 16; ks++) {
+        const uint64_t hdesc = make_smem_desc(gam + ks * 256,  128,  512);
+        const uint64_t ldesc = make_smem_desc(gam + kNCL * kTE * 2 + ks * 256, 128, 512);
+        const uint64_t sdesc = make_smem_desc(gam + 2 * kNCL * kTE * 2 + ks * 256, 128, 512);
+#if GMM_MSTEP_CUT == 1
+        asm volatile("" ::"r"(hi[ks][0]), "r"(hi[ks][1]), "r"(hi[ks][2]), "r"(hi[ks][3]), "r"(lo[ks][0]), "r"(lo[ks][1]), "r"(lo[ks][2]),
+                     "r"(lo[ks][3]), "l"(hdesc), "l"(ldesc), "l"(sdesc));
+        (void)ex; (void)rm; (void)new1; (void)new2;
+#else
+        wgmma_m64n32k16_rs(ex, hi[ks][0], hi[ks][1], hi[ks][2], hi[ks][3], hdesc, ks > 0 || !new1);
+        wgmma_m64n32k16_rs(rm, hi[ks][0], hi[ks][1], hi[ks][2], hi[ks][3], ldesc, ks > 0 || !new2);
+        wgmma_m64n32k16_rs(rm, lo[ks][0], lo[ks][1], lo[ks][2], lo[ks][3], sdesc, true);
+#endif
+    }
 }
 
 __device__ __forceinline__ bool chain_ends(int i, int mt, int nsub) { return ((i + mt) % kChunkSub) == kChunkSub - 1 || i == nsub - 1; }
@@ -152,7 +150,7 @@
 template <int D>
 __global__ void __launch_bounds__(MCfg<D>::THREADS, 1)
 mstep_tc_kernel(const __grid_constant__ CUtensorMap tm_x, const __grid_constant__ CUtensorMap tm_g, int n,
-                float* __restrict__ scratch, int events_per_cta, const __grid_constant__ MMagic magic) {
+                float* __restrict__ scratch, int events_per_cta, const __grid_constant__ MMagic magic, const int* __restrict__ opmap) {
     using C = MCfg<D>;
     extern __shared__ __align__(1024) uint8_t smem[];
     uint64_t* bars = reinterpret_cast<uint64_t*>(smem + C::OFF_BAR);
@@ -167,13 +165,13 @@
     const int nsub = (e_end - e_begin + kTE - 1) / kTE;
     const int k0 = blockIdx.y * kNCL;
 
-    for (int i = threadIdx.x * 16; i < C::OFF_RAWX; i += C::THREADS * 16) *reinterpret_cast<uint4*>(smem + i) = make_uint4(0, 0, 0, 0);
+    for (int i = threadIdx.x; i < kNRAW * 256; i += C::THREADS)
+        reinterpret_cast<float*>(smem + C::OFF_RAWX + (i >> 8) * C::RAWX + C::RAWZ)[i & 255] = 1.0f;
     if (threadIdx.x == 0) {
-        for (int s = 0; s < kNRAW; s++) { mbar_init(&raw_full[s], 1); mbar_init(&raw_empty[s], 4); }
-        for (int s = 0; s < kNST; s++) { mbar_init(&op_full[s], 4); mbar_init(&op_empty[s], 4 * C::MT); }
+        for (int s = 0; s < kNRAW; s++) { mbar_init(&raw_full[s], 1); mbar_init(&raw_empty[s], 3 + 4 * C::MT); }
+        for (int s = 0; s < kNST; s++) { mbar_init(&op_full[s], 3); mbar_init(&op_empty[s], 4 * C::MT); }
         fence_mbar_init();
     }
-    fence_proxy_async_smem();
     __syncthreads();
 
     if (warp < 4) {
@@ -189,111 +187,124 @@
                     tma_load_2d(smem + C::OFF_RAWG + st * C::RAWG, &tm_g, e0, k0, &raw_full[st]);
                 }
             }
-        }
-    } else if (warp < 12) {
-        set_regs<C::REG_B, C::REG_LAUNCH>();
-        const int bwg = (warp - 4) >> 2;
-        const int part = (warp - 4) & 3;
-        const int bt = threadIdx.x - 128 - bwg * 128;
-        for (int i = bwg; i < nsub; i += 2) {
+        } else {
+            const int bt = threadIdx.x - 32;
+            constexpr int NIT = 2;
+            for (int i = 0; i < nsub; i++) {
+                const int rs = i % kNRAW, rph = (i / kNRAW) & 1;
+                const int os = i % kNST, oph = (i / kNST) & 1;
+                mbar_wait_parked(&raw_full[rs], rph, 200);
+                uint4 gh[NIT], gl[NIT], gs[NIT];
+                float dep = 0.0f;
+#pragma unroll
+                for (int u = 0; u < NIT; u++) {
+                    const int it = bt + 96 * u;
+                    if (it >= 128) break;
+                    const int kg = it >> 5, l = it & 31;
+                    const int k = kg * 8 + (l & 7), ce = l >> 3;
+                    const uint8_t* grow = smem + C::OFF_RAWG + rs * C::RAWG + k * (kTE * 4);
+                    const float4 a = *reinterpret_cast<const float4*>(grow + (((2 * ce) ^ (k & 7)) << 4));
+                    const float4 b = *reinterpret_cast<const float4*>(grow + (((2 * ce + 1) ^ (k & 7)) << 4));
+                    const float g[8] = {a.x, a.y, a.z, a.w, b.x, b.y, b.z, b.w};
+                    dep += a.x + b.x;
+                    float hi[8], lo[8];
+#pragma unroll
+                    for (int v = 0; v < 8; v++) {
+                        hi[v] = __fsub_rn(__fmaf_rn(g[v], kGammaScale, kGammaMagic), kGammaMagic);
+                        lo[v] = __fmaf_rn(g[v], kGammaScale, -hi[v]);
+                    }
+                    gh[u] = make_uint4(pack_half2(hi[0], hi[1]), pack_half2(hi[2], hi[3]), pack_half2(hi[4], hi[5]), pack_half2(hi[6], hi[7]));
+                    gl[u] = make_uint4(pack_half2(lo[0], lo[1]), pack_half2(lo[2], lo[3]), pack_half2(lo[4], lo[5]), pack_half2(lo[6], lo[7]));
+                    gs[u] = make_uint4(pack_half2(g[0] * kGammaScale, g[1] * kGammaScale), pack_half2(g[2] * kGammaScale, g[3] * kGammaScale),
+                                       pack_half2(g[4] * kGammaScale, g[5] * kGammaScale), pack_half2(g[6] * kGammaScale, g[7] * kGammaScale));
+                }
+                __syncwarp();
+                if (lane == 0) mbar_arrive_after(&raw_empty[rs], dep);
+                else asm volatile("" ::"f"(dep));
+                mbar_wait_parked(&op_empty[os], oph ^ 1, 200);
+                uint8_t* g_hi = smem + C::OFF_G + os * C::G_STAGE;
+#pragma unroll
+                for (int u = 0; u < NIT; u++) {
+                    const int it = bt + 96 * u;
+                    if (it >= 128) break;
+                    const int kg = it >> 5, l = it & 31;
+                    *reinterpret_cast<uint4*>(g_hi + kg * 512 + l * 16) = gh[u];
+                    *reinterpret_cast<uint4*>(g_hi + C::G_PART + kg * 512 + l * 16) = gl[u];
+                    *reinterpret_cast<uint4*>(g_hi + 2 * C::G_PART + kg * 512 + l * 16) = gs[u];
+                }
+                fence_proxy_async_smem();
+                __syncwarp();
+                if (lane == 0) mbar_arrive(&op_full[os]);
+            }
+        }
+    } else {
+        set_regs<C::REG_C, C::REG_LAUNCH>();
+        const int mt = __shfl_sync(0xffffffffu, (warp - 4) >> 2, 0);
+        const int ct = threadIdx.x - 128;
+        const int wq = warp & 3, gid = lane >> 2, qd = lane & 3;
+        float* racc = reinterpret_cast<float*>(smem + C::OFF_RACC) + ct;
+#pragma unroll
+        for (int j = 0; j < 32; j++) racc[j * C::NCT] = 0.0f;
+        uint32_t fa, fb[4];
+        float mg[4];
+        {
+            const int* om = opmap + mt * 128 + wq * 16 + gid;
+            auto addr = [&](int code) {
+                const uint32_t row = code >= kRowOne ? (uint32_t)(C::RAWZ / 128 + code - kRowOne) : (uint32_t)code;
+                return row * 128 + ((((uint32_t)qd >> 1) ^ (row & 7)) << 4) + ((uint32_t)qd & 1) * 8;
+            };
+#pragma unroll
+            for (int s = 0; s < 4; s++) {
+                const int c = om[(s >> 1) * 64 + (s & 1) * 8];
+                const int a = c & 255, b = c >> 8;
+                if (s == 0) fa = addr(a);
+                fb[s] = addr(b);
+                mg[s] = a >= kRowOne && b >= kRowOne ? 0.0f : (a >= kRowOne || b >= kRowOne ? magic.lin : magic.prod);
+            }
+        }
+        const uint32_t zs0 = smem_u32(smem + C::OFF_RAWX);
+        float ex[2][16], rm[2][16];
+#pragma unroll
+        for (int h = 0; h < 2; h++)
+#pragma unroll
+            for (int j = 0; j < 16; j++) { ex[h][j] = 0.0f; rm[h][j] = 0.0f; }
+        uint32_t fh[2][2][4], fl[2][2][4];
+        int held = -1;
+        for (int i = 0; i < nsub; i++) {
             const int rs = i % kNRAW, rph = (i / kNRAW) & 1;
             const int os = i % kNST, oph = (i / kNST) & 1;
-            mbar_wait_parked(&raw_full[rs], rph, 200);
-            float z[D];
-            {
-                const float* xr = reinterpret_cast<const float*>(smem + C::OFF_RAWX + rs * C::RAWX) + lane;
-                int dd = part * C::S;
-#pragma unroll
-                for (int d = 0; d < D; d++) { z[d] = xr[dd * kTE]; dd = dd + 1 == D ? 0 : dd + 1; }
-            }
-            uint4 gh, gl, gs;
-            float gdep;
-            {
-                const int kg = bt >> 5, l = bt & 31;
-                const int k = kg * 8 + (l & 7), ce = l >> 3;
-                const uint8_t* grow = smem + C::OFF_RAWG + rs * C::RAWG + k * (kTE * 4);
-                const float4 a = *reinterpret_cast<const float4*>(grow + (((2 * ce) ^ (k & 7)) << 4));
-                const float4 b = *reinterpret_cast<const float4*>(grow + (((2 * ce + 1) ^ (k & 7)) << 4));
-                const float g[8] = {a.x, a.y, a.z, a.w, b.x, b.y, b.z, b.w};
-                gdep = a.x + b.x;
-                float hi[8], lo[8];
-#pragma unroll
-                for (int u = 0; u < 8; u++) {
-                    hi[u] = __fsub_rn(__fmaf_rn(g[u], kGammaScale, kGammaMagic), kGammaMagic);
-                    lo[u] = __fmaf_rn(g[u], kGammaScale, -hi[u]);
-                }
-                gh = make_uint4(pack_half2(hi[0], hi[1]), pack_half2(hi[2], hi[3]), pack_half2(hi[4], hi[5]), pack_half2(hi[6], hi[7]));
-                gl = make_uint4(pack_half2(lo[0], lo[1]), pack_half2(lo[2], lo[3]), pack_half2(lo[4], lo[5]), pack_half2(lo[6], lo[7]));
-                gs = make_uint4(pack_half2(g[0] * kGammaScale, g[1] * kGammaScale), pack_half2(g[2] * kGammaScale, g[3] * kGammaScale),
-                                pack_half2(g[4] * kGammaScale, g[5] * kGammaScale), pack_half2(g[6] * kGammaScale, g[7] * kGammaScale));
-            }
-            float dep = gdep;
-#pragma unroll
-            for (int d = 0; d < D; d++) dep += z[d];
-            __syncwarp();
-            if (lane == 0) mbar_arrive_after(&raw_empty[rs], dep);
-            else asm volatile("" ::"f"(dep));
-            mbar_wait_parked(&op_empty[os], oph ^ 1, 200);
-            uint8_t* phi_hi = smem + C::OFF_PHI + os * C::PHI_STAGE;
-            uint8_t* phi_lo = phi_hi + C::PHI_PART;
-            build_phi_chunks<D>(z, magic, phi_hi, phi_lo, lane, part);
-            {
-                uint8_t* g_hi = smem + C::OFF_G + os * C::G_STAGE;
-                const int kg = bt >> 5, l = bt & 31;
-                *reinterpret_cast<uint4*>(g_hi + kg * 512 + l * 16) = gh;
-                *reinterpret_cast<uint4*>(g_hi + C::G_PART + kg * 512 + l * 16) = gl;
-                *reinterpret_cast<uint4*>(g_hi + 2 * C::G_PART + kg * 512 + l * 16) = gs;
-            }
-            fence_proxy_async_smem();
-            __syncwarp();
-            if (lane == 0) mbar_arrive(&op_full[os]);
-        }
-    } else {
-        set_regs<C::REG_C, C::REG_LAUNCH>();
-        const int mt = __shfl_sync(0xffffffffu, (warp - 12) >> 2, 0);
-        const int ct = threadIdx.x - 384;
-        const int wq = warp & 3, gid = lane >> 2, qd = lane & 3;
-        float* racc = reinterpret_cast<float*>(smem + C::OFF_RACC) + ct;
-#pragma unroll
-        for (int j = 0; j < 32; j++) racc[j * C::NCT] = 0.0f;
-        float ex[2][16], rm[2][16];
-#pragma unroll
-        for (int h = 0; h < 2; h++)
-#pragma unroll
-            for (int j = 0; j < 16; j++) { ex[h][j] = 0.0f; rm[h][j] = 0.0f; }
-        int held = -1;
-        for (int i = 0; i < nsub; i++) {
-            const int os = i % kNST, oph = (i / kNST) & 1;
-            mbar_wait_parked(&op_full[os], oph, 100);
-            const uint32_t phi = smem_u32(smem + C::OFF_PHI + os * C::PHI_STAGE);
+            const uint32_t zst = zs0 + rs * C::RAWX;
             const uint32_t gam = smem_u32(smem + C::OFF_G + os * C::G_STAGE);
             const bool new1 = chain_starts(i, mt), new2 = chain2_starts(i, mt);
+            mbar_wait_parked(&raw_full[rs], rph, 100);
+            float2 za[4], zb0[4], zb1[4];
+            load_row(zst + fa, za);
+            load_row(zst + fb[0], zb0);
+            load_row(zst + fb[1], zb1);
+            build_half(za, zb0, zb1, mg[0], mg[1], fh[0], fl[0]);
+            mbar_wait_parked(&op_full[os], oph, 100);
             wgmma_fence();
-#pragma unroll
-            for (int h = 0; h < 2; h++) {
-#pragma unroll
-                for (int ks = 0; ks < kTE / 16; ks++) {
-                    const uint64_t hdesc = make_smem_desc(gam + ks * 256,  128,  512);
-                    const uint64_t ldesc = make_smem_desc(gam + C::G_PART + ks * 256, 128, 512);
-                    const uint64_t sdesc = make_smem_desc(gam + 2 * C::G_PART + ks * 256, 128, 512);
-                    const uint32_t arow = mt * 8192 + h * 4096 + ks * 256;
-                    const uint64_t ah = make_smem_desc(phi + arow,  128,  512);
-                    const uint64_t al = make_smem_desc(phi + C::PHI_PART + arow, 128, 512);
-                    wgmma_m64n32k16_ss_tn(ex[h], ah, hdesc, ks > 0 || !new1);
-                    wgmma_m64n32k16_ss_tn(rm[h], ah, ldesc, ks > 0 || !new2);
-                    wgmma_m64n32k16_ss_tn(rm[h], al, sdesc);
-                }
-            }
+            issue_half(ex[0], rm[0], fh[0], fl[0], gam, new1, new2);
             wgmma_commit();
             wgmma_wait<1>();
             __syncwarp();
             if (lane == 0 && held >= 0) mbar_arrive(&op_empty[held]);
+            load_row(zst + fb[2], zb0);
+            load_row(zst + fb[3], zb1);
+            build_half(za, zb0, zb1, mg[2], mg[3], fh[1], fl[1]);
+            wgmma_fence();
+            issue_half(ex[1], rm[1], fh[1], fl[1], gam, new1, new2);
+            wgmma_commit();
+            __syncwarp();
+            if (lane == 0) mbar_arrive(&raw_empty[rs]);
+            wgmma_wait<1>();
             held = os;
             if (chain_ends(i, mt, nsub)) {
                 wgmma_wait<0>();
                 __syncwarp();
                 if (lane == 0) mbar_arrive(&op_empty[os]);
                 held = -1;
+#if GMM_MSTEP_CUT != 3
 #pragma unroll
                 for (int h = 0; h < 2; h++) {
 #pragma unroll
@@ -308,9 +319,16 @@
                         asm volatile("" ::: "memory");
                     }
                 }
+#endif
             }
         }
         wgmma_wait<0>();
+#if GMM_MSTEP_CUT == 3
+#pragma unroll
+        for (int h = 0; h < 2; h++)
+#pragma unroll
+            for (int j = 0; j < 16; j++) racc[(h * 16 + j) * C::NCT] += ex[h][j] + rm[h][j];
+#endif
         float* my = scratch + (size_t)(blockIdx.y * gridDim.x + blockIdx.x) * C::MT * 128 * kNCL + (size_t)mt * 128 * kNCL;
 #pragma unroll
         for (int h = 0; h < 2; h++)
@@ -789,6 +807,7 @@
     float zmax[GMM_MAX_DIMENSIONS] = {0};
     MMagic magic{0.f, 0.f};
     int3* d_rowmap = nullptr;
+    int* d_opmap = nullptr;
     CUtensorMap tm_cx{}, tm_cg{};
     const void* cmap_z = nullptr;
     const void* cmap_g = nullptr;
@@ -863,7 +882,7 @@
     TC_CUDA_TRY(cudaMalloc(&t->d_inv_scale_f, sizeof(float) * GMM_MAX_DIMENSIONS));
     TC_CUDA_TRY(cudaMalloc(&t->d_scale, sizeof(double) * GMM_MAX_DIMENSIONS));
     TC_CUDA_TRY(cudaMalloc(&t->d_z_soa, sizeof(float) * memb_pitch * D));
-    if (int rc = make_map_2d(&t->tm_x, t->d_z_soa, (uint64_t)n, (uint64_t)D, (uint64_t)memb_pitch * 4, kTE, (uint32_t)D)) return rc;
+    if (int rc = make_map_2d(&t->tm_x, t->d_z_soa, (uint64_t)n, (uint64_t)D, (uint64_t)memb_pitch * 4, kTE, (uint32_t)D, true)) return rc;
     if (int rc = make_map_2d(&t->tm_g, d_memb, (uint64_t)n, (uint64_t)Kmax, (uint64_t)memb_pitch * 4, kTE, kNCL, true)) return rc;
     t->maps_ok = true;
     if (D == 8 || D == 16 || D == 24) {
@@ -881,22 +900,27 @@
         if (passes > 1) TC_CUDA_TRY(cudaMalloc(&t->d_den, sizeof(float) * memb_pitch));
         t->emap_ok = true;
     }
-    const int rpp = 1 + 2 * (D / 4) + (D / 4) * (D / 2), nrows = 4 * ((rpp + 7) / 8) * 8;
-    const int mt = (nrows + 127) / 128;
+    const int mt = mstep_tiles(D);
     {
-        std::vector<int3> rm((size_t)mt * 128);
+        const std::vector<MRow> rows = mstep_row_layout(D);
+        if (rows.size() != (size_t)mt * 128) return fail(GMM_ERR_STATE, "tensor M-step row map: the statistics do not fit the feature tiles");
+        std::vector<int3> rm(rows.size());
+        std::vector<int> om(rows.size());
         std::vector<char> seen((size_t)num_features(D), 0);
-        for (int row = 0; row < mt * 128; row++) {
-            const RowInfo ri = tc_row_info(D, row);
-            rm[row] = make_int3(ri.f, ri.i, ri.j);
-            if (ri.f >= 0) {
-                if (seen[ri.f]) return fail(GMM_ERR_STATE, "tensor M-step row map: a statistic is produced twice");
-                seen[ri.f] = 1;
+        for (size_t row = 0; row < rows.size(); row++) {
+            const MRow& r = rows[row];
+            rm[row] = make_int3(r.f, r.i, r.j);
+            om[row] = r.a | r.b << 8;
+            if (r.f >= 0) {
+                if (seen[r.f]) return fail(GMM_ERR_STATE, "tensor M-step row map: a statistic is produced twice");
+                seen[r.f] = 1;
             }
         }
         for (char c : seen) if (!c) return fail(GMM_ERR_STATE, "tensor M-step row map: a statistic is not produced");
         TC_CUDA_TRY(cudaMalloc(&t->d_rowmap, sizeof(int3) * rm.size()));
         TC_CUDA_TRY(cudaMemcpy(t->d_rowmap, rm.data(), sizeof(int3) * rm.size(), cudaMemcpyHostToDevice));
+        TC_CUDA_TRY(cudaMalloc(&t->d_opmap, sizeof(int) * om.size()));
+        TC_CUDA_TRY(cudaMemcpy(t->d_opmap, om.data(), sizeof(int) * om.size(), cudaMemcpyHostToDevice));
     }
     const int ytiles = (Kmax + kNCL - 1) / kNCL;
     t->scratch_floats = (size_t)num_sms * ytiles * mt * 128 * kNCL;
@@ -916,7 +940,7 @@
 void tc_destroy(TcState* t) {
     if (!t) return;
     cudaFree(t->d_shift_f); cudaFree(t->d_inv_scale_f); cudaFree(t->d_scale); cudaFree(t->d_scratch);
-    cudaFree(t->d_opnd); cudaFree(t->d_den); cudaFree(t->d_z_soa); cudaFree(t->d_rowmap);
+    cudaFree(t->d_opnd); cudaFree(t->d_den); cudaFree(t->d_z_soa); cudaFree(t->d_rowmap); cudaFree(t->d_opmap);
     if (t->h_opnd) cudaFreeHost(t->h_opnd);
     if (t->ev_h2d) cudaEventDestroy(t->ev_h2d);
     delete t;
@@ -1489,9 +1513,9 @@
     const int gy = (K + kNCL - 1) / kNCL;
     if ((size_t)gx * gy * C::MT * 128 * kNCL > t->scratch_floats) return fail(GMM_ERR_STATE, "tensor M-step scratch too small");
     dim3 grid(gx, gy);
-    mstep_tc_kernel<D><<<grid, C::THREADS, C::SMEM_BYTES, stream>>>(tm_x, tm_g, n, t->d_scratch, per, t->magic);
+    mstep_tc_kernel<D><<<grid, C::THREADS, C::SMEM_BYTES, stream>>>(tm_x, tm_g, n, t->d_scratch, per, t->magic, t->d_opmap);
     TC_CUDA_TRY(cudaGetLastError());
-    mstep_tc_finalize_kernel<<<C::NCHUNK * 8, 256, 0, stream>>>(t->d_scratch, gx, C::MT, K, C::F, t->d_rowmap, t->d_scale, d_stats);
+    mstep_tc_finalize_kernel<<<C::MT * 128, 256, 0, stream>>>(t->d_scratch, gx, C::MT, K, C::F, t->d_rowmap, t->d_scale, d_stats);
     TC_CUDA_TRY(cudaGetLastError());
     return GMM_OK;
 }
@@ -1521,7 +1545,7 @@
     if (!t || !t->maps_ok) return fail(GMM_ERR_STATE, "tensor-core M-step not initialised for this shape");
     if (t->cmap_z != d_z || t->cmap_g != d_memb || t->cmap_pitch != pitch || t->cmap_n != n) {
         t->cmap_n = -1;
-        if (int rc = make_map_2d(&t->tm_cx, d_z, (uint64_t)n, (uint64_t)t->D, (uint64_t)pitch * 4, kTE, (uint32_t)t->D)) return rc;
+        if (int rc = make_map_2d(&t->tm_cx, d_z, (uint64_t)n, (uint64_t)t->D, (uint64_t)pitch * 4, kTE, (uint32_t)t->D, true)) return rc;
         if (int rc = make_map_2d(&t->tm_cg, d_memb, (uint64_t)n, (uint64_t)t->Kmax, (uint64_t)pitch * 4, kTE, kNCL, true)) return rc;
         t->cmap_z = d_z; t->cmap_g = d_memb; t->cmap_pitch = pitch; t->cmap_n = n;
     }
diff --git a/cuda-gmm-mpi_b200/csrc/mstep_rows.h b/cuda-gmm-mpi_b200/csrc/mstep_rows.h
--- /dev/null
+++ b/cuda-gmm-mpi_b200/csrc/mstep_rows.h
@@ -0,0 +1,171 @@
+#pragma once
+#include <algorithm>
+#include <array>
+#include <vector>
+
+namespace gmm {
+
+constexpr int kRowOne = 32;
+
+struct MRow {
+    int f, i, j;
+    int a, b;
+};
+
+inline int mstep_feat2(int D, int i, int j) { return 1 + D + i * (i + 1) / 2 + j; }
+
+inline int mstep_tiles(int D) {
+    const int S = D / 4, rpp = 1 + 2 * S + S * (D / 2), rows = 4 * ((rpp + 7) / 8) * 8;
+    return (rows + 127) / 128;
+}
+
+inline std::vector<int> mstep_stat_tiles(int D) {
+    const int S = D / 4, half = D / 2, rpp = 1 + 2 * S + S * half, cpp = (rpp + 7) / 8;
+    std::vector<int> tile(1 + D + D * (D + 1) / 2, -1);
+    for (int row = 0; row < 4 * cpp * 8; row++) {
+        const int p = row / (cpp * 8), r = row % (cpp * 8);
+        int f = -1;
+        if (r >= rpp) continue;
+        if (r == 0) f = p == 0 ? 0 : -1;
+        else if (r <= S) f = 1 + (r - 1 + p * S) % D;
+        else {
+            int a, b;
+            if (r <= 2 * S) a = b = r - 1 - S;
+            else { const int t = r - 1 - 2 * S; a = t / half; b = (a + 1 + t % half) % D; }
+            const int ta = (a + p * S) % D, tb = (b + p * S) % D;
+            if (!(a != b && (b - a + D) % D == half && ta >= half)) f = mstep_feat2(D, std::max(ta, tb), std::min(ta, tb));
+        }
+        if (f >= 0) tile[f] = row / 128;
+    }
+    return tile;
+}
+
+inline std::vector<MRow> mstep_row_layout(int D) {
+    const int MT = mstep_tiles(D);
+    const std::vector<int> tile = mstep_stat_tiles(D);
+    std::vector<MRow> out((size_t)MT * 128, MRow{-1, -1, -1, kRowOne, kRowOne});
+    constexpr int ONE = -1;
+    struct Item { int f, i, j, o0, o1; };
+    auto cls = [](int r) { return (r >> 1) & 3; };
+    for (int mt = 0; mt < MT; mt++) {
+        std::vector<Item> items;
+        for (int f = 0; f < (int)tile.size(); f++) {
+            if (tile[f] != mt) continue;
+            if (f == 0) items.push_back({f, -1, -1, ONE, -2});
+            else if (f <= D) items.push_back({f, f - 1, -1, f - 1, ONE});
+            else {
+                int i = 0;
+                while ((i + 1) * (i + 2) / 2 <= f - 1 - D) i++;
+                const int j = f - 1 - D - i * (i + 1) / 2;
+                items.push_back({f, i, j, i, i == j ? -2 : j});
+            }
+        }
+        std::vector<char> done(items.size(), 0), closed(D + 1, 0);
+        std::vector<std::pair<int, std::vector<int>>> groups;
+        for (;;) {
+            std::vector<std::vector<int>> cand(D + 1);
+            for (int k = 0; k < (int)items.size(); k++) {
+                if (done[k]) continue;
+                for (int o : {items[k].o0, items[k].o1})
+                    if (o != -2 && !closed[o + 1]) cand[o + 1].push_back(k);
+            }
+            int best = -1;
+            for (int g = 0; g <= D; g++)
+                if (!cand[g].empty() && (best < 0 || cand[g].size() < cand[best].size())) best = g;
+            if (best < 0) break;
+            const int fac = best - 1;
+            std::vector<int> forced, flex;
+            for (int k : cand[best]) {
+                const int other = items[k].o0 == fac ? items[k].o1 : items[k].o0;
+                (other == -2 || closed[other + 1] ? forced : flex).push_back(k);
+            }
+            int m = (int)cand[best].size() / 4 * 4;
+            if (m < (int)forced.size()) m = std::min((int)cand[best].size(), ((int)forced.size() + 3) / 4 * 4);
+            auto other_cands = [&](int k) {
+                const int other = items[k].o0 == fac ? items[k].o1 : items[k].o0;
+                return (int)cand[other + 1].size();
+            };
+            std::stable_sort(flex.begin(), flex.end(), [&](int x, int y) { return other_cands(x) > other_cands(y); });
+            std::vector<int> take = forced;
+            for (int k = 0; k < (int)flex.size() && (int)take.size() < m; k++) take.push_back(flex[k]);
+            for (size_t q = 0; q < take.size(); q += 4)
+                groups.push_back({fac, std::vector<int>(take.begin() + q, take.begin() + std::min(take.size(), q + 4))});
+            for (int k : take) done[k] = 1;
+            closed[best] = 1;
+        }
+        if (groups.size() > 32) return {};
+        std::stable_sort(groups.begin(), groups.end(), [](const auto& x, const auto& y) {
+            return (x.first == ONE ? 1000 : x.first) < (y.first == ONE ? 1000 : y.first);
+        });
+        while (groups.size() < 32) groups.push_back({ONE, {}});
+        for (int w = 0; w < 4; w++) {
+            std::array<std::vector<int>, 4> slot_rows;
+            std::array<std::array<int, 4>, 8> bsel{};
+            std::array<std::array<int, 4>, 8> fsel{};
+            std::array<int, 8> asel{};
+            for (int gid = 0; gid < 8; gid++) {
+                const auto& g = groups[gid * 4 + w];
+                asel[gid] = g.first;
+                std::array<int, 4> bs{ONE, ONE, ONE, ONE}, fs{-1, -1, -1, -1};
+                for (size_t u = 0; u < g.second.size(); u++) {
+                    const Item& it = items[g.second[u]];
+                    fs[u] = it.f;
+                    if (it.f == 0) bs[u] = ONE;
+                    else if (it.j < 0) bs[u] = g.first == ONE ? it.i : ONE;
+                    else bs[u] = g.first == it.i ? it.j : it.i;
+                }
+                auto waves = [&](const std::vector<int>& rows) {
+                    int c[4] = {0, 0, 0, 0};
+                    std::vector<int> seen;
+                    for (int r : rows)
+                        if (r != ONE && std::find(seen.begin(), seen.end(), r) == seen.end()) { seen.push_back(r); c[cls(r)]++; }
+                    return *std::max_element(c, c + 4);
+                };
+                std::array<int, 4> perm{0, 1, 2, 3}, best_perm = perm;
+                int best_cost = 1 << 30;
+                do {
+                    int cost = 0;
+                    for (int s = 0; s < 4; s++) {
+                        std::vector<int> rows = slot_rows[s];
+                        rows.push_back(bs[perm[s]]);
+                        cost += waves(rows);
+                    }
+                    if (cost < best_cost) { best_cost = cost; best_perm = perm; }
+                } while (std::next_permutation(perm.begin(), perm.end()));
+                for (int s = 0; s < 4; s++) {
+                    slot_rows[s].push_back(bs[best_perm[s]]);
+                    bsel[gid][s] = bs[best_perm[s]];
+                    fsel[gid][s] = fs[best_perm[s]];
+                }
+            }
+            auto one_code = [&](const std::vector<int>& rows) {
+                int c[4] = {0, 0, 0, 0};
+                std::vector<int> seen;
+                for (int r : rows)
+                    if (r != ONE && std::find(seen.begin(), seen.end(), r) == seen.end()) { seen.push_back(r); c[cls(r)]++; }
+                return kRowOne + 2 * (int)(std::min_element(c, c + 4) - c);
+            };
+            const int a_one = one_code(std::vector<int>(asel.begin(), asel.end()));
+            for (int s = 0; s < 4; s++) {
+                const int b_one = one_code(slot_rows[s]);
+                for (int gid = 0; gid < 8; gid++) {
+                    MRow& o = out[(size_t)mt * 128 + (s >> 1) * 64 + w * 16 + gid + 8 * (s & 1)];
+                    o.a = asel[gid] == ONE ? a_one : asel[gid];
+                    o.b = bsel[gid][s] == ONE ? b_one : bsel[gid][s];
+                    const int f = fsel[gid][s];
+                    if (f < 0) continue;
+                    o.f = f;
+                    if (f == 0) continue;
+                    if (f <= D) { o.i = f - 1; continue; }
+                    const Item* it = nullptr;
+                    for (const Item& x : items) if (x.f == f) it = &x;
+                    o.i = it->i;
+                    o.j = it->j;
+                }
+            }
+        }
+    }
+    return out;
+}
+
+}
diff --git a/cuda-gmm-mpi_b200/csrc/tc_ptx.cuh b/cuda-gmm-mpi_b200/csrc/tc_ptx.cuh
--- a/cuda-gmm-mpi_b200/csrc/tc_ptx.cuh
+++ b/cuda-gmm-mpi_b200/csrc/tc_ptx.cuh
@@ -90,6 +90,17 @@
         : "r"(a0), "r"(a1), "r"(a2), "r"(a3), "l"(b_desc), "r"((uint32_t)accumulate));
 }
 
+__device__ __forceinline__ void wgmma_m64n32k16_rs(float (&d)[16], uint32_t a0, uint32_t a1, uint32_t a2, uint32_t a3, uint64_t b_desc, bool accumulate) {
+    asm volatile(
+        "{\n\t.reg .pred p;\n\t"
+        "setp.ne.b32 p, %21, 0;\n\t"
+        "wgmma.mma_async.sync.aligned.m64n32k16.f32.f16.f16 "
+        "{%0, %1, %2, %3, %4, %5, %6, %7, %8, %9, %10, %11, %12, %13, %14, %15}, "
+        "{%16, %17, %18, %19}, %20, p, 1, 1, 0;\n\t}"
+        : "+f"(d[0]), "+f"(d[1]), "+f"(d[2]), "+f"(d[3]), "+f"(d[4]), "+f"(d[5]), "+f"(d[6]), "+f"(d[7]), "+f"(d[8]), "+f"(d[9]), "+f"(d[10]), "+f"(d[11]), "+f"(d[12]), "+f"(d[13]), "+f"(d[14]), "+f"(d[15])
+        : "r"(a0), "r"(a1), "r"(a2), "r"(a3), "l"(b_desc), "r"((uint32_t)accumulate));
+}
+
 __device__ __forceinline__ void wgmma_m64n32k16_ss_tn(float (&d)[16], uint64_t a_desc, uint64_t b_desc, bool accumulate = true) {
     asm volatile(
         "{\n\t.reg .pred p;\n\t"
```

New measurement: 126.5 (median of 6 runs). 5.0% higher.
